# brownvc/matryodshka

Measured on AMD Instinct MI355X. Metric: novel-view frames/sec, 640x320 ODS->32-sphere MSI infer+render, higher is better.
Workload: dtype f32

## Files before the change

### include/msi_hip.h

```cpp
#ifndef MSI_HIP_H
#define MSI_HIP_H

#include <stddef.h>
#include <stdint.h>

#ifdef __cplusplus
extern "C" {
#endif

#define MSI_OK 0
#define MSI_E_BADARG (-1)
#define MSI_E_LAUNCH (-2)
#define MSI_E_UNSUPPORTED (-3)
#define MSI_E_WORKSPACE (-4)
#define MSI_E_RANGE (-5)

typedef void *msi_stream_t;

const char *msi_version(void);
#define MSI_ABI_VERSION 9
int32_t msi_abi_version(void);
const char *msi_last_error_string(void);
uint32_t msi_crc32c_host(const void *data_host, size_t n, uint32_t crc);

int32_t msi_probe_matrix_rate(int32_t changing_operands, int64_t iterations, int32_t num_workgroups, uint64_t *ticks_device, float *sink_device,
                              msi_stream_t stream);

size_t msi_trig_table_floats(int32_t height, int32_t width);
int msi_build_trig_tables_host(int32_t height, int32_t width, float *out_host);

int msi_preprocess_u8_f32(const uint8_t *in, float *out, size_t n, msi_stream_t stream);
int msi_preprocess_f32(const float *in, float *out, size_t n, msi_stream_t stream);
int msi_preprocess_pair_u8_f32(const uint8_t *in0, const uint8_t *in1, float *out0, float *out1, size_t n,
                               msi_stream_t stream);
int msi_deprocess_f32_u8(const float *in, uint8_t *out, size_t n, int32_t is_depth,
                         msi_stream_t stream);
int msi_deprocess_pair_f32_u8(const float *rgb, const float *depth, uint8_t *out_rgb, uint8_t *out_depth, size_t n,
                              msi_stream_t stream);

int msi_compose_poses_f32(const float *lhs, const float *rhs, float *out, int32_t batch,
                          msi_stream_t stream);

int msi_ods_sphere_sweep_f32(const float *image, const float *pose, const float *intrinsics,
                             const float *depths, const float *trig, int32_t batch,
                             int32_t height, int32_t width, int32_t num_depths, int32_t order,
                             float *psv, int32_t psv_channels, int32_t channel_offset,
                             msi_stream_t stream);

int msi_ods_sphere_sweep_bf16(const float *image, const float *pose, const float *intrinsics,
                              const float *depths, const float *trig, int32_t batch,
                              int32_t height, int32_t width, int32_t num_depths, int32_t order,
                              void *psv_bf16, int32_t psv_channels, int32_t channel_offset,
                              msi_stream_t stream);

int msi_ods_sweep_volume(const float *ref_image, const float *src_image, const float *ref_curr_pose,
                         const float *src_curr_pose, const float *intrinsics, const float *depths, const float *trig,
                         int32_t batch, int32_t height, int32_t width, int32_t num_depths, void *psv, int32_t psv_is_bf16,
                         msi_stream_t stream);
int msi_compose_pose_pair_f32(const float *lhs0, const float *lhs1, const float *rhs, float *out0, float *out1,
                              int32_t batch, msi_stream_t stream);

int msi_assemble_rgba_f32(const float *psv, const float *pred, float *rgba_native,
                          float *blend_weights, float *alphas, int32_t batch, int32_t height,
                          int32_t width, int32_t num_planes, msi_stream_t stream);

int msi_assemble_rgba_bf16psv_f32(const void *psv_bf16, const float *pred, float *rgba_native,
                                  float *blend_weights, float *alphas, int32_t batch, int32_t height,
                                  int32_t width, int32_t num_planes, msi_stream_t stream);

#define MSI_COLOR_BLEND_PSV 0
#define MSI_COLOR_BLEND_BG 1
#define MSI_COLOR_BLEND_BG_PSV 2
#define MSI_COLOR_ALPHA_ONLY 3
int msi_assemble_rgba_color_f32(const void *psv, int32_t psv_is_bf16, const float *pred, int32_t which_color_pred,
                                float *rgba_native, float *blend_weights, float *alphas, float *bg_blend_weights,
                                int32_t batch, int32_t height, int32_t width, int32_t num_planes, msi_stream_t stream);

int msi_resize_bilinear_f32(const float *in, float *out, int32_t batch, int32_t in_h, int32_t in_w,
                            int32_t channels, int32_t out_h, int32_t out_w, msi_stream_t stream);
int msi_assemble_rgba_scaled_f32(const float *psv, const float *weights_alphas, float *rgba_native,
                                 int32_t batch, int32_t height, int32_t width, int32_t num_planes,
                                 msi_stream_t stream);
int msi_hres_layers(const float *ref_image, const float *src_image, const float *ref_curr_pose, const float *src_curr_pose,
                    const float *intrinsics, const float *depths, const float *trig, const float *blend_weights,
                    const float *alphas, int32_t batch, int32_t low_height, int32_t low_width, int32_t height, int32_t width,
                    int32_t num_planes, float *rgba_native, void *layers_out, int32_t format, msi_stream_t stream);

#define MSI_RENDER_STATUS_ORIGIN_OUTSIDE 1
int msi_render_equirect_f32(const float *rgba_native, const float *tgt_pose_rt,
                            const float *tgt_pos, const float *depths, const float *trig,
                            int32_t batch, int32_t height, int32_t width, int32_t num_planes,
                            float *out_rgb, float *out_depth, int32_t *status_device, msi_stream_t stream);
#define MSI_CAMERA_EQUIRECT 0
#define MSI_CAMERA_PINHOLE 1
int msi_render_views_f32(const float *rgba_native, const float *tgt_pose_rt, const float *tgt_pos,
                         const float *intrinsics, const float *depths, const float *trig,
                         int32_t batch, int32_t views, int32_t height, int32_t width, int32_t num_planes,
                         int32_t camera, int32_t out_height, int32_t out_width,
                         float *out_rgb, float *out_depth, int32_t *status_device, msi_stream_t stream);

#define MSI_LAYERS_F32 0
#define MSI_LAYERS_RGBA8 1
#define MSI_LAYERS_RGBA16F 2
int msi_pack_layers(const float *rgba_native, int32_t format, void *packed, int64_t texels, msi_stream_t stream);
int msi_unpack_layers(const void *packed, int32_t format, float *rgba_native, int64_t texels, msi_stream_t stream);
int msi_render_views_packed(const void *layers, int32_t format, const float *tgt_pose_rt, const float *tgt_pos,
                            const float *intrinsics, const float *depths, const float *trig,
                            int32_t batch, int32_t views, int32_t height, int32_t width, int32_t num_planes,
                            int32_t camera, int32_t out_height, int32_t out_width,
                            float *out_rgb, float *out_depth, int32_t *status_device, msi_stream_t stream);
int msi_render_ods_views(const void *layers, int32_t format, const float *tgt_pose_rt, const float *tgt_pos,
                         const float *eye_radius, const float *depths, const float *trig,
                         int32_t batch, int32_t views, int32_t height, int32_t width, int32_t num_planes,
                         int32_t out_height, int32_t out_width,
                         float *out_rgb, float *out_depth, int32_t *status_device, msi_stream_t stream);
int msi_sparse_index_tiles(const void *layers, int32_t format, int32_t batch, int32_t num_planes, int32_t height, int32_t width,
                           int32_t *table_out, int32_t *counts_out, msi_stream_t stream);
int msi_sparse_gather_tiles(const void *layers, int32_t format, const int32_t *table, const int64_t *layer_start, int32_t batch,
                            int32_t num_planes, int32_t height, int32_t width, void *pool_out, msi_stream_t stream);
int msi_sparse_expand(const void *pool, const int32_t *table, const int64_t *layer_start, int32_t format, int32_t batch,
                      int32_t num_planes, int32_t height, int32_t width, void *layers_out, msi_stream_t stream);
int msi_render_views_sparse(const void *pool, const int32_t *table, const int64_t *layer_start, int32_t format,
                            const float *tgt_pose_rt, const float *tgt_pos, const float *intrinsics, const float *eye_radius,
                            const float *depths, const float *trig, int32_t batch, int32_t views, int32_t height, int32_t width,
                            int32_t num_planes, int32_t camera, int32_t out_height, int32_t out_width, float *out_rgb,
                            float *out_depth, int32_t *status_device, msi_stream_t stream);
int msi_hres_index_tiles(const float *alphas, int32_t format, int32_t batch, int32_t low_height, int32_t low_width,
                         int32_t height, int32_t width, int32_t num_planes,
                         int32_t *table_out, int32_t *counts_out, msi_stream_t stream);
int msi_hres_layers_sparse(const float *ref_image, const float *src_image, const float *ref_curr_pose, const float *src_curr_pose,
                           const float *intrinsics, const float *depths, const float *trig, const float *blend_weights,
                           const float *alphas, int32_t batch, int32_t low_height, int32_t low_width, int32_t height, int32_t width,
                           int32_t num_planes, const int32_t *table, const int64_t *layer_start, void *pool_out, int32_t format,
                           msi_stream_t stream);
int msi_project_layers_f32(const float *rgba_native, const float *tgt_pose_rt,
                           const float *tgt_pos, const float *depths, const float *trig,
                           int32_t batch, int32_t height, int32_t width, int32_t num_planes,
                           float *out_layers, int32_t *status_device, msi_stream_t stream);

int msi_render_ods_f32(const float *rgba_native, const float *pose, const float *intrinsics,
                       const float *depths, const float *trig, int32_t batch, int32_t height,
                       int32_t width, int32_t num_planes, int32_t order, float *out_rgb,
                       int32_t *status_device, msi_stream_t stream);
int msi_render_perspective_f32(const float *rgba_native, const float *pose, const float *tgt_pos,
                               const float *depths, int32_t batch, int32_t height, int32_t width,
                               int32_t num_planes, int32_t tgt_height, int32_t tgt_width, float *out_rgb,
                               int32_t *status_device, msi_stream_t stream);

int msi_perspective_plane_sweep_f32(const float *image, const float *pose, const float *intrinsics,
                                    const float *depths, int32_t batch, int32_t height, int32_t width,
                                    int32_t num_depths, float *psv, int32_t psv_channels,
                                    int32_t channel_offset, msi_stream_t stream);
int msi_perspective_sweep_volume_bf16(const float *ref_image, const float *src_image, const float *ref_curr_pose,
                                      const float *src_curr_pose, const float *intrinsics, const float *depths,
                                      int32_t batch, int32_t height, int32_t width, int32_t num_depths,
                                      void *psv_bf16, msi_stream_t stream);
int msi_mpi_render_f32(const float *rgba_native, const float *tgt_pose, const float *intrinsics,
                       const float *intrinsics_inv, const float *depths, int32_t batch, int32_t height,
                       int32_t width, int32_t num_planes, float *out_rgb, msi_stream_t stream);
int msi_mpi_render_views(const void *layers, int32_t format, const float *tgt_pose, const float *intrinsics,
                         const float *tgt_intrinsics_inv, const float *depths, int32_t batch, int32_t views, int32_t height,
                         int32_t width, int32_t num_planes, int32_t out_height, int32_t out_width, float *out_rgb,
                         float *out_depth, msi_stream_t stream);

int msi_cube_render_views(const void *layers, int32_t format, const float *tgt_pose_rt, const float *tgt_pos,
                          const float *tgt_intrinsics, const float *stack_intrinsics, const float *depths, const float *trig,
                          int32_t batch, int32_t views, int32_t face_size, int32_t num_planes, int32_t camera,
                          int32_t out_height, int32_t out_width, float *out_rgb, float *out_depth, int32_t *status_device,
                          msi_stream_t stream);
int msi_equirect_to_cube_f32(const float *image, const float *intrinsics, int32_t batch, int32_t height, int32_t width,
                             int32_t channels, int32_t face_size, float *out, msi_stream_t stream);

#define MSI_SCORE_F32 0
#define MSI_SCORE_U8 1
#define MSI_SCORE_RAW 0
#define MSI_SCORE_IMAGE 1
#define MSI_SCORE_DEPTH 2
#define MSI_SCORE_MSE 1u
#define MSI_SCORE_MAE 2u
#define MSI_SCORE_SSIM 4u
size_t msi_score_workspace_bytes(int32_t n_pairs, int32_t height, int32_t width, int32_t channels);
int msi_score_images(const void *pred, const void *target, int32_t dtype, int32_t transform, int32_t quantize, int32_t n_pairs,
                     int32_t group, int32_t height, int32_t width, int32_t channels, const double *row_weights, double max_val,
                     uint32_t metrics, double *out, void *workspace, size_t workspace_bytes, msi_stream_t stream);

typedef struct msi_net_desc {
  int32_t batch, height, width;
  int32_t in_channels;
  int32_t num_outputs;
  int32_t ngf;
  int32_t coord_net;
  int32_t dtype;
} msi_net_desc;

#define MSI_DTYPE_F32 0
#define MSI_DTYPE_BF16 1

#define MSI_NET_NUM_LAYERS 18

typedef struct msi_layer_info {
  char name[16];
  int32_t kind;
  int32_t cin, cout;
  int32_t has_coord;
  int32_t stride, rate;
  int32_t in_h, in_w, out_h, out_w;
  uint64_t param_offset;
  uint64_t param_floats;
  uint64_t raw_offset;
  uint64_t affine_offset;
  uint64_t ln_scale_offset;
} msi_layer_info;

int msi_net_layer_info(const msi_net_desc *desc, int32_t layer, msi_layer_info *out);
size_t msi_net_param_floats(const msi_net_desc *desc);
size_t msi_net_packed_floats(const msi_net_desc *desc);
int msi_net_pack_weights_host(const msi_net_desc *desc, const float *params_host,
                              float *packed_host);
size_t msi_net_workspace_bytes(const msi_net_desc *desc);

typedef struct msi_net_plan msi_net_plan;
#define MSI_NET_OPT_FIXUP_KERNEL 0
#define MSI_NET_OPT_TAILSPLIT 1
#define MSI_NET_OPT_BIGTILE 2
#define MSI_NET_OPT_HEAD_FUSE_LN 3
#define MSI_NET_OPT_NUM_CUS 4
#define MSI_NET_OPT_F32_TILE 5
#define MSI_NET_OPT_F32_TILE_MASK 6
#define MSI_NET_OPT_APPLY_AHEAD 7
#define MSI_NET_OPT_HALO 8
#define MSI_NET_OPT_HALO_SKIP 9
#define MSI_NET_OPT_UNIFORM_SPLIT 10
#define MSI_NET_OPT_BF16_STAGE_RAW 11
#define MSI_NET_OPT_SPLIT_OVERHEAD 12
#define MSI_NET_OPT_BF16_WAVES 13
#define MSI_NET_OPT_F32_SPLIT3 14
#define MSI_NET_OPT_F32_SPLIT_F16 15
#define MSI_NET_OPT_X3_TILE8 16
#define MSI_NET_OPT_X3_ROWPAR 17
#define MSI_NET_OPT_COUNT 18
int msi_net_plan_create(const msi_net_desc *desc, msi_net_plan **out_plan);
void msi_net_plan_destroy(msi_net_plan *plan);
int msi_net_plan_set_option(msi_net_plan *plan, int32_t option, int32_t value);
size_t msi_net_plan_workspace_bytes(const msi_net_plan *plan);
int32_t msi_net_plan_layer_is_normalized(const msi_net_plan *plan, int32_t layer);
int32_t msi_net_plan_layer_kernel(const msi_net_plan *plan, int32_t layer, char *name, size_t name_bytes, int32_t *nblocks,
                                  int32_t *nsplit_tiles);
int32_t msi_net_plan_layer_params(const msi_net_plan *plan, int32_t layer, void *out, size_t bytes, size_t *needed);
#define MSI_NET_STATUS_APPLY_AHEAD_TIMEOUT 1
#define MSI_NET_STATUS_LN_OVERFLOW 2
#define MSI_NET_STATUS_LN_UNDERFLOW 4
#define MSI_NET_STATUS_F16_SPLIT_RANGE 8
int32_t msi_net_plan_status(const msi_net_plan *plan, const void *workspace, msi_stream_t stream, int32_t *status_bits);
int32_t msi_net_plan_calibrate(const msi_net_plan *plan, float *packed, const void *net_input, void *workspace, size_t workspace_bytes,
                               msi_stream_t stream, int32_t *layers_changed);
int msi_net_plan_forward(const msi_net_plan *plan, const float *packed, const void *net_input, float *pred,
                         void *workspace, size_t workspace_bytes, msi_stream_t stream);

int msi_net_plan_forward_rgba(const msi_net_plan *plan, const float *packed, const void *net_input, float *rgba_native,
                              float *blend_weights, float *alphas, float *pred, void *workspace, size_t workspace_bytes,
                              msi_stream_t stream, void *event_after_convs);

int msi_net_plan_forward_layers(const msi_net_plan *plan, const float *packed, const void *net_input, float *rgba_native,
                                void *layers_out, int32_t format, float *blend_weights, float *alphas, float *pred,
                                void *workspace, size_t workspace_bytes, msi_stream_t stream, void *event_after_convs);

int msi_net_forward_f32(const msi_net_desc *desc, const float *packed, const float *net_input,
                        float *pred, void *workspace, size_t workspace_bytes,
                        msi_stream_t stream);
int msi_net_forward_bf16(const msi_net_desc *desc, const float *packed, const void *net_input_bf16,
                         float *pred, void *workspace, size_t workspace_bytes,
                         msi_stream_t stream);

#ifdef __cplusplus
}
#endif
#endif
```

### matryodshka_amd/_native.py

```python
import ctypes
import os
from ctypes import POINTER, Structure, c_char, c_char_p, c_float, c_int32, c_size_t, c_uint64, c_void_p

_HERE = os.path.dirname(os.path.abspath(__file__))
LIB_PATH = os.path.join(_HERE, "libmsi_hip.so")

MSI_OK = 0
MSI_NET_NUM_LAYERS = 18
RENDER_STATUS_ORIGIN_OUTSIDE = 1
MSI_CAMERA_EQUIRECT, MSI_CAMERA_PINHOLE = 0, 1
MSI_LAYERS_F32, MSI_LAYERS_RGBA8, MSI_LAYERS_RGBA16F = 0, 1, 2
MSI_SCORE_F32, MSI_SCORE_U8 = 0, 1
MSI_SCORE_RAW, MSI_SCORE_IMAGE, MSI_SCORE_DEPTH = 0, 1, 2
MSI_SCORE_MSE, MSI_SCORE_MAE, MSI_SCORE_SSIM = 1, 2, 4
MSI_ABI_VERSION = 9


class MsiError(RuntimeError):
    pass


class NetDesc(Structure):
    _fields_ = [("batch", c_int32), ("height", c_int32), ("width", c_int32),
                ("in_channels", c_int32), ("num_outputs", c_int32), ("ngf", c_int32),
                ("coord_net", c_int32), ("dtype", c_int32)]


MSI_DTYPE_F32, MSI_DTYPE_BF16 = 0, 1
NET_OPT_FIXUP_KERNEL, NET_OPT_TAILSPLIT, NET_OPT_BIGTILE, NET_OPT_HEAD_FUSE_LN, NET_OPT_NUM_CUS = 0, 1, 2, 3, 4
NET_OPT_F32_TILE, NET_OPT_F32_TILE_MASK, NET_OPT_APPLY_AHEAD, NET_OPT_HALO, NET_OPT_HALO_SKIP = 5, 6, 7, 8, 9
NET_OPT_UNIFORM_SPLIT, NET_OPT_BF16_STAGE_RAW, NET_OPT_SPLIT_OVERHEAD, NET_OPT_BF16_WAVES, NET_OPT_F32_SPLIT3 = 10, 11, 12, 13, 14
NET_OPT_F32_SPLIT_F16 = 15
NET_OPT_X3_TILE8 = 16
NET_OPT_X3_ROWPAR = 17
NET_STATUS_F16_SPLIT_RANGE = 8


class LayerInfo(Structure):
    _fields_ = [("name", c_char * 16), ("kind", c_int32), ("cin", c_int32), ("cout", c_int32),
                ("has_coord", c_int32), ("stride", c_int32), ("rate", c_int32),
                ("in_h", c_int32), ("in_w", c_int32), ("out_h", c_int32), ("out_w", c_int32),
                ("param_offset", c_uint64), ("param_floats", c_uint64),
                ("raw_offset", c_uint64), ("affine_offset", c_uint64), ("ln_scale_offset", c_uint64)]


_P = c_void_p
_I = c_int32

SIGNATURES = {
    "msi_version": (c_char_p, []),
    "msi_abi_version": (c_int32, []),
    "msi_last_error_string": (c_char_p, []),
    "msi_crc32c_host": (ctypes.c_uint32, [_P, c_size_t, ctypes.c_uint32]),
    "msi_probe_matrix_rate": (_I, [_I, ctypes.c_int64, _I, _P, _P, _P]),
    "msi_trig_table_floats": (c_size_t, [_I, _I]),
    "msi_build_trig_tables_host": (_I, [_I, _I, _P]),
    "msi_preprocess_u8_f32": (_I, [_P, _P, c_size_t, _P]),
    "msi_preprocess_pair_u8_f32": (_I, [_P, _P, _P, _P, c_size_t, _P]),
    "msi_deprocess_pair_f32_u8": (_I, [_P, _P, _P, _P, c_size_t, _P]),
    "msi_preprocess_f32": (_I, [_P, _P, c_size_t, _P]),
    "msi_deprocess_f32_u8": (_I, [_P, _P, c_size_t, _I, _P]),
    "msi_compose_poses_f32": (_I, [_P, _P, _P, _I, _P]),
    "msi_ods_sphere_sweep_f32": (_I, [_P, _P, _P, _P, _P, _I, _I, _I, _I, _I, _P, _I, _I, _P]),
    "msi_ods_sphere_sweep_bf16": (_I, [_P, _P, _P, _P, _P, _I, _I, _I, _I, _I, _P, _I, _I, _P]),
    "msi_ods_sweep_volume": (_I, [_P, _P, _P, _P, _P, _P, _P, _I, _I, _I, _I, _P, _I, _P]),
    "msi_compose_pose_pair_f32": (_I, [_P, _P, _P, _P, _P, _I, _P]),
    "msi_assemble_rgba_f32": (_I, [_P, _P, _P, _P, _P, _I, _I, _I, _I, _P]),
    "msi_assemble_rgba_bf16psv_f32": (_I, [_P, _P, _P, _P, _P, _I, _I, _I, _I, _P]),
    "msi_assemble_rgba_color_f32": (_I, [_P, _I, _P, _I, _P, _P, _P, _P, _I, _I, _I, _I, _P]),
    "msi_resize_bilinear_f32": (_I, [_P, _P, _I, _I, _I, _I, _I, _I, _P]),
    "msi_assemble_rgba_scaled_f32": (_I, [_P, _P, _P, _I, _I, _I, _I, _P]),
    "msi_hres_layers": (_I, [_P, _P, _P, _P, _P, _P, _P, _P, _P, _I, _I, _I, _I, _I, _I, _P, _P, _I, _P]),
    "msi_render_equirect_f32": (_I, [_P, _P, _P, _P, _P, _I, _I, _I, _I, _P, _P, _P, _P]),
    "msi_render_views_f32": (_I, [_P, _P, _P, _P, _P, _P, _I, _I, _I, _I, _I, _I, _I, _I, _P, _P, _P, _P]),
    "msi_pack_layers": (_I, [_P, _I, _P, ctypes.c_int64, _P]),
    "msi_unpack_layers": (_I, [_P, _I, _P, ctypes.c_int64, _P]),
    "msi_render_views_packed": (_I, [_P, _I, _P, _P, _P, _P, _P, _I, _I, _I, _I, _I, _I, _I, _I, _P, _P, _P, _P]),
    "msi_render_ods_views": (_I, [_P, _I, _P, _P, _P, _P, _P, _I, _I, _I, _I, _I, _I, _I, _P, _P, _P, _P]),
    "msi_sparse_index_tiles": (_I, [_P, _I, _I, _I, _I, _I, _P, _P, _P]),
    "msi_sparse_gather_tiles": (_I, [_P, _I, _P, _P, _I, _I, _I, _I, _P, _P]),
    "msi_sparse_expand": (_I, [_P, _P, _P, _I, _I, _I, _I, _I, _P, _P]),
    "msi_render_views_sparse": (_I, [_P, _P, _P, _I, _P, _P, _P, _P, _P, _P, _I, _I, _I, _I, _I, _I, _I, _I, _P, _P, _P, _P]),
    "msi_hres_index_tiles": (_I, [_P, _I, _I, _I, _I, _I, _I, _I, _P, _P, _P]),
    "msi_hres_layers_sparse": (_I, [_P, _P, _P, _P, _P, _P, _P, _P, _P, _I, _I, _I, _I, _I, _I, _P, _P, _P, _I, _P]),
    "msi_project_layers_f32": (_I, [_P, _P, _P, _P, _P, _I, _I, _I, _I, _P, _P, _P]),
    "msi_render_ods_f32": (_I, [_P, _P, _P, _P, _P, _I, _I, _I, _I, _I, _P, _P, _P]),
    "msi_render_perspective_f32": (_I, [_P, _P, _P, _P, _I, _I, _I, _I, _I, _I, _P, _P, _P]),
    "msi_perspective_plane_sweep_f32": (_I, [_P, _P, _P, _P, _I, _I, _I, _I, _P, _I, _I, _P]),
    "msi_perspective_sweep_volume_bf16": (_I, [_P, _P, _P, _P, _P, _P, _I, _I, _I, _I, _P, _P]),
    "msi_mpi_render_f32": (_I, [_P, _P, _P, _P, _P, _I, _I, _I, _I, _P, _P]),
    "msi_mpi_render_views": (_I, [_P, _I, _P, _P, _P, _P, _I, _I, _I, _I, _I, _I, _I, _P, _P, _P]),
    "msi_cube_render_views": (_I, [_P, _I, _P, _P, _P, _P, _P, _P, _I, _I, _I, _I, _I, _I, _I, _P, _P, _P, _P]),
    "msi_equirect_to_cube_f32": (_I, [_P, _P, _I, _I, _I, _I, _I, _P, _P]),
    "msi_score_workspace_bytes": (c_size_t, [_I, _I, _I, _I]),
    "msi_score_images": (_I, [_P, _P, _I, _I, _I, _I, _I, _I, _I, _I, _P, ctypes.c_double, ctypes.c_uint32, _P, _P, c_size_t, _P]),
    "msi_net_layer_info": (_I, [POINTER(NetDesc), _I, POINTER(LayerInfo)]),
    "msi_net_param_floats": (c_size_t, [POINTER(NetDesc)]),
    "msi_net_packed_floats": (c_size_t, [POINTER(NetDesc)]),
    "msi_net_pack_weights_host": (_I, [POINTER(NetDesc), _P, _P]),
    "msi_net_workspace_bytes": (c_size_t, [POINTER(NetDesc)]),
    "msi_net_plan_create": (_I, [POINTER(NetDesc), POINTER(c_void_p)]),
    "msi_net_plan_destroy": (None, [_P]),
    "msi_net_plan_set_option": (_I, [_P, _I, _I]),
    "msi_net_plan_workspace_bytes": (c_size_t, [_P]),
    "msi_net_plan_layer_is_normalized": (_I, [_P, _I]),
    "msi_net_plan_layer_kernel": (_I, [_P, _I, _P, c_size_t, POINTER(c_int32), POINTER(c_int32)]),
    "msi_net_plan_layer_params": (_I, [_P, _I, _P, c_size_t, POINTER(c_size_t)]),
    "msi_net_plan_status": (_I, [_P, _P, _P, POINTER(c_int32)]),
    "msi_net_plan_calibrate": (_I, [_P, _P, _P, _P, c_size_t, _P, POINTER(c_int32)]),
    "msi_net_plan_forward": (_I, [_P, _P, _P, _P, _P, c_size_t, _P]),
    "msi_net_plan_forward_rgba": (_I, [_P, _P, _P, _P, _P, _P, _P, _P, c_size_t, _P, _P]),
    "msi_net_plan_forward_layers": (_I, [_P, _P, _P, _P, _P, _I, _P, _P, _P, _P, c_size_t, _P, _P]),
    "msi_net_forward_f32": (_I, [POINTER(NetDesc), _P, _P, _P, _P, c_size_t, _P]),
    "msi_net_forward_bf16": (_I, [POINTER(NetDesc), _P, _P, _P, _P, c_size_t, _P]),
}


def _load():
    import torch
    if not os.path.exists(LIB_PATH):
        raise ImportError(
            "matryodshka_amd: %s is missing -- build it with `python -m matryodshka_amd.build` "
            "(or __graft_entry__.build()).  There is no CPU fallback." % LIB_PATH)
    lib = ctypes.CDLL(LIB_PATH)
    for name, (res, args) in SIGNATURES.items():
        try:
            fn = getattr(lib, name)
        except AttributeError:
            raise ImportError("matryodshka_amd: %s does not export %s" % (LIB_PATH, name))
        fn.restype = res
        fn.argtypes = args
    if lib.msi_abi_version() != MSI_ABI_VERSION:
        raise ImportError("matryodshka_amd: %s has ABI version %d, this binding is written for %d -- rebuild it "
                          "(python -m matryodshka_amd.build --force)" % (LIB_PATH, lib.msi_abi_version(), MSI_ABI_VERSION))
    return lib


lib = _load()


def last_error():
    return lib.msi_last_error_string().decode("utf-8", "replace")


class NetPlan(object):

    def __init__(self, desc, options=None):
        h = c_void_p()
        check(lib.msi_net_plan_create(desc, ctypes.byref(h)), "msi_net_plan_create")
        self.handle = h
        self._destroy = lib.msi_net_plan_destroy
        for key, value in (options or {}).items():
            self.set_option(key, value)

    def set_option(self, key, value):
        check(lib.msi_net_plan_set_option(self.handle, int(key), int(value)), "msi_net_plan_set_option")

    def workspace_bytes(self):
        return lib.msi_net_plan_workspace_bytes(self.handle)

    def layer_kernel(self, layer):
        buf = ctypes.create_string_buffer(96)
        nb, ns = c_int32(0), c_int32(0)
        check(lib.msi_net_plan_layer_kernel(self.handle, int(layer), ctypes.cast(buf, c_void_p), 96, ctypes.byref(nb), ctypes.byref(ns)),
              "msi_net_plan_layer_kernel")
        return buf.value.decode(), int(nb.value), int(ns.value)

    def layer_params(self, layer):
        n = c_size_t(0)
        check(lib.msi_net_plan_layer_params(self.handle, int(layer), None, 0, ctypes.byref(n)), "msi_net_plan_layer_params")
        buf = ctypes.create_string_buffer(n.value)
        check(lib.msi_net_plan_layer_params(self.handle, int(layer), ctypes.cast(buf, c_void_p), n.value, None), "msi_net_plan_layer_params")
        return buf.raw

    def kernels(self):
        return [self.layer_kernel(i) for i in range(18)]

    def __del__(self):
        h, self.handle = getattr(self, "handle", None), None
        if h:
            self._destroy(h)


def check(rc, what):
    if rc != MSI_OK:
        raise MsiError("%s failed (code %d): %s" % (what, rc, last_error()))
```

### matryodshka_amd/csrc/cnn.hip

```cpp
#include "cnn_plan.h"

namespace msi_cnn {

int device_cu_count() {
  int dev = 0;
  hipDeviceProp_t prop;
  if (hipGetDevice(&dev) != hipSuccess || hipGetDeviceProperties(&prop, dev) != hipSuccess || prop.multiProcessorCount <= 0) {
    (void)hipGetLastError();
    return DEFAULT_CUS;
  }
  return prop.multiProcessorCount;
}

int launch_conv(const LayerLaunch &Q, const ConvParams &p, hipStream_t stream) {
  const ConvVariant &V = Q.variant;
  int rc;
  switch (V.family) {
    case CONV_IGEMM: rc = launch_igemm(Q, p, stream); break;
    case CONV_HALO: case CONV_HALO_S2: case CONVT_HALO: rc = launch_halo_f32(Q, p, stream); break;
    case CONV_HALO_X3: case CONV_HALO8_X3: case CONV_HALO_S2_X3: case CONV_HALO8_S2_X3: case CONVT_HALO_X3: case CONVT_HALO8_X3: rc = launch_x3(Q, p, stream); break;
    case CONV_HALO_BF16: case CONV_HALO_BF16_S2: case CONVT_HALO_BF16: rc = launch_bf16_halo(Q, p, stream); break;
    default: return msi::fail(MSI_E_UNSUPPORTED, "conv: unknown kernel family %d", V.family);
  }
  if (rc || Q.nfix == 0 || p.tile_cnt != nullptr) return rc;
  const int mode = V.family == CONV_IGEMM ? V.mode : (V.is_convt() ? MODE_CONVT : MODE_CONV);
  return launch_fixup(V.bm, V.bn, mode, V.family == CONV_IGEMM && V.bf16 && mode != MODE_HEAD, Q.nfix, V.is_convt() ? 2 : 1, p, stream);
}

}

#if defined(MSI_CONV_TIMING) || defined(MSI_DEBUG_STATS)
static unsigned long long *g_timing_buf = nullptr;
static int g_timing_layer = -1;
extern "C" int msi_debug_conv_occupancy(int lds_bytes) {
  return msi_cnn::debug_conv_occupancy(lds_bytes);
}
extern "C" void msi_debug_conv_timing(void *device_buffer, int layer) {
  g_timing_buf = static_cast<unsigned long long *>(device_buffer);
  g_timing_layer = layer;
}
#endif

extern "C" {

#ifdef MSI_DEBUG_SUMS
extern "C" long long msi_debug_sums_offset(const msi_net_plan *plan, int layer) { return (long long)plan->net.layers[layer].sums_off; }
extern "C" long long msi_debug_partial_offset(const msi_net_plan *plan) { return (long long)plan->net.partial_off; }
#endif
static int run_layers(const msi_net_plan *plan, const float *packed, const void *net_input, float *pred,
                      void *workspace, size_t workspace_bytes, msi_stream_t stream_, int nlayers) {
  MSI_REQUIRE(plan, "net_forward: null plan");
  const msi_net_desc *desc = &plan->desc;
  const Net &net = plan->net;
  const int bf16 = desc->dtype == MSI_DTYPE_BF16;
  MSI_REQUIRE(packed && net_input && workspace, "net_forward: null pointer");
  if (workspace_bytes < net.ws_bytes)
    return msi::fail(MSI_E_WORKSPACE, "net_forward: workspace %zu B < required %zu B", workspace_bytes,
                     net.ws_bytes);
  if (desc->batch == 0) return MSI_OK;
  hipStream_t stream = msi::as_stream(stream_);
  char *ws = static_cast<char *>(workspace);
  {
    const size_t n16 = net.zero_bytes / 16;
    int rc0 = launch_zero(ws + net.zero_off, n16, stream);
    if (rc0) return rc0;
  }
  int *cnt = reinterpret_cast<int *>(ws + net.cnt_off);
  for (int li = 0; li < nlayers; ++li) {
    const Layer &L = net.layers[li];
    const LayerLaunch &Q = plan->launch[li];
    ConvParams p = Q.p;
    auto src_ptr = [&](int s) -> const char * {
      if (s < 0) return static_cast<const char *>(net_input);
      return ws + (bf16 ? net.layers[s].act_off : net.layers[s].raw_off);
    };
    p.x0 = src_ptr(L.src0);
    p.x1 = L.src1 >= 0 ? src_ptr(L.src1) : p.x0;
    p.wpk = reinterpret_cast<const char *>(packed + L.packed_off);
    p.coord_bias = L.has_coord ? packed + L.coord_off : nullptr;
    p.bias = L.kind == MODE_HEAD ? packed + L.gamma_off : nullptr;
    if (Q.fuse_ln) {
      const Layer &S = net.layers[L.src0];
      p.ln_sums = reinterpret_cast<const long long *>(ws + S.sums_off);
      p.ln_gamma = packed + S.gamma_off;
      p.ln_beta = packed + S.beta_off;
    }
    p.y = L.kind == MODE_HEAD ? pred : reinterpret_cast<float *>(ws + L.raw_off);
    p.sums = L.kind == MODE_HEAD ? nullptr : reinterpret_cast<long long *>(ws + L.sums_off);
    auto scl_of = [&](int li2) { return reinterpret_cast<const double *>(packed + net.layers[li2].lnscl_off); };
    p.ln_scl = L.kind == MODE_HEAD ? nullptr : scl_of(li);
    p.ln_scl_src = L.src0 >= 0 ? scl_of(L.src0) : nullptr;
    p.ln_scl_src1 = L.src1 >= 0 ? scl_of(L.src1) : nullptr;
    p.status = reinterpret_cast<int *>(ws + net.err_off);
    p.partial = reinterpret_cast<float *>(ws + net.partial_off);
    p.tile_cnt = Q.inlaunch ? cnt + (size_t)li * CONV_SLOTS_PER_CU * plan->num_cus : nullptr;
#if defined(MSI_CONV_TIMING) || defined(MSI_DEBUG_STATS)
    p.dbg = (li == g_timing_layer) ? g_timing_buf : nullptr;
#endif
    auto raw_source = [&](int s, bool second) {
      const Layer &S = net.layers[s];
      if (!second) {
        if (bf16) p.x0 = ws + S.raw_off;
        p.ln_sums = reinterpret_cast<const long long *>(ws + S.sums_off); p.ln_gamma = packed + S.gamma_off; p.ln_beta = packed + S.beta_off;
      } else {
        if (bf16) p.x1 = ws + S.raw_off;
        p.ln_sums1 = reinterpret_cast<const long long *>(ws + S.sums_off); p.ln_gamma1 = packed + S.gamma_off; p.ln_beta1 = packed + S.beta_off;
      }
    };
    const ConvVariant &V = Q.variant;
    if (V.is_convt()) {
      if (p.halo_apply & 1) raw_source(L.src0, false);
      if (p.halo_apply & 2) raw_source(L.src1, true);
    } else if (V.apply) {
      raw_source(L.src0, false);
    }
    if (V.six_product()) p.wpk_x3 = reinterpret_cast<const char *>(packed + (V.planes == 2 ? L.x2_off : L.x3_off));
    int rc = launch_conv(Q, p, stream);
    if (rc) return rc;
    const bool tail_src = bf16 && nlayers == MSI_NET_NUM_LAYERS - 1 && li == net.layers[MSI_NET_NUM_LAYERS - 1].src0;
    if (L.kind != MODE_HEAD && !Q.skip_apply && !tail_src) {
      const size_t per_sample = (size_t)L.out_h * L.out_w * L.cout;
      float *raw = reinterpret_cast<float *>(ws + L.raw_off), *aff = reinterpret_cast<float *>(ws + L.aff_off);
      const size_t lds = (size_t)2 * L.cout * sizeof(float);
      const long long *sums = reinterpret_cast<const long long *>(ws + L.sums_off);
      rc = launch_ln_apply(bf16, Q.ln_blocks, desc->batch, lds, stream, raw, sums, 1.0 / L.ln_count, scl_of(li), p.status, packed + L.gamma_off, packed + L.beta_off,
                           per_sample, L.cout, aff, bf16 ? reinterpret_cast<unsigned short *>(ws + L.act_off) : static_cast<unsigned short *>(nullptr));
      if (rc) return rc;
    }
  }
  return MSI_OK;
}

int32_t msi_net_plan_status(const msi_net_plan *plan, const void *workspace, msi_stream_t stream_, int32_t *status_bits) {
  MSI_REQUIRE(plan && workspace, "net_plan_status: null pointer");
  hipStream_t stream = msi::as_stream(stream_);
  int word = 0;
  hipError_t e = hipMemcpyAsync(&word, static_cast<const char *>(workspace) + plan->net.err_off, sizeof(int), hipMemcpyDeviceToHost, stream);
  if (e == hipSuccess) e = hipStreamSynchronize(stream);
  if (e != hipSuccess) return msi::fail(MSI_E_LAUNCH, "net_plan_status: %s", hipGetErrorString(e));
  if (status_bits) *status_bits = word;
  if (word == 0) return MSI_OK;
  return msi::fail(MSI_E_RANGE, "net_plan_status: 0x%x:%s%s%s", word,
                   (word & STATUS_F16_SPLIT_RANGE) ? " an operand of a layer on the fp16 split exceeded the fp16 range (|x| > 65504): set MSI_NET_OPT_F32_SPLIT_F16 = 0" : "",
                   (word & STATUS_LN_OVERFLOW) ? " a LayerNorm sum left its fixed-point window (raw convolution output far above the scale the weights predict: non-finite or mis-scaled input?)" : "",
                   (word & STATUS_LN_UNDERFLOW) ? " a LayerNorm variance is below the resolution of its fixed-point window (raw convolution output far below the scale the weights predict, or constant)" : "");
}

int32_t msi_net_plan_calibrate(const msi_net_plan *plan, float *packed, const void *net_input, void *workspace, size_t workspace_bytes,
                               msi_stream_t stream_, int32_t *layers_changed) {
  MSI_REQUIRE(plan && packed && net_input && workspace, "net_plan_calibrate: null pointer");
  const Net &net = plan->net;
  const msi_net_desc *desc = &plan->desc;
  hipStream_t stream = msi::as_stream(stream_);
  if (layers_changed) *layers_changed = 0;
  if (desc->batch == 0) return MSI_OK;
  const size_t nwords = (size_t)desc->batch * LN_SHARDS * LN_WORDS;
  std::vector<long long> sums(nwords);
  char *ws = static_cast<char *>(workspace);
  constexpr int NL = MSI_NET_NUM_LAYERS - 1;
  double orig[NL][LN_SCL_DOUBLES];
  hipError_t he = hipSuccess;
  for (int li = 0; li < NL && he == hipSuccess; ++li)
    he = hipMemcpyAsync(orig[li], packed + net.layers[li].lnscl_off, sizeof(orig[li]), hipMemcpyDeviceToHost, stream);
  if (he == hipSuccess) he = hipStreamSynchronize(stream);
  if (he != hipSuccess) return msi::fail(MSI_E_LAUNCH, "net_plan_calibrate: %s", hipGetErrorString(he));
  int touched = 0;
  auto restore = [&]() {
    for (int l = 0; l < touched; ++l)
      (void)hipMemcpyAsync(packed + net.layers[l].lnscl_off, orig[l], sizeof(orig[l]), hipMemcpyHostToDevice, stream);
    (void)hipStreamSynchronize(stream);
  };
  for (int li = 0; li < NL; ++li) {
    const Layer &L = net.layers[li];
    const double *scl = orig[li];
    int e0 = LN_S1_BITS - (int)lrint(log2(scl[0])), e = e0;
    bool settled = false;
    touched = li + 1;
    for (int it = 0; it < 24 && !settled; ++it) {
      const double ns[LN_SCL_DOUBLES] = {ldexp(1.0, LN_S1_BITS - e), ldexp(1.0, LN_S2_BITS - 2 * e), ldexp(1.0, -(LN_S1_BITS - e)), ldexp(1.0, -(LN_S2_BITS - 2 * e))};
      he = hipMemcpyAsync(packed + L.lnscl_off, ns, sizeof(ns), hipMemcpyHostToDevice, stream);
      if (he == hipSuccess) he = hipStreamSynchronize(stream);
      if (he != hipSuccess) { restore(); return msi::fail(MSI_E_LAUNCH, "net_plan_calibrate: %s", hipGetErrorString(he)); }
      int rc = run_layers(plan, packed, net_input, nullptr, workspace, workspace_bytes, stream_, li + 1);
      if (rc) { restore(); return rc; }
      int word = 0;
      he = hipMemcpyAsync(sums.data(), ws + L.sums_off, nwords * sizeof(long long), hipMemcpyDeviceToHost, stream);
      if (he == hipSuccess) he = hipMemcpyAsync(&word, ws + net.err_off, sizeof(int), hipMemcpyDeviceToHost, stream);
      if (he == hipSuccess) he = hipStreamSynchronize(stream);
      if (he != hipSuccess) { restore(); return msi::fail(MSI_E_LAUNCH, "net_plan_calibrate: %s", hipGetErrorString(he)); }
      if (word & STATUS_LN_OVERFLOW) { e += 12; if (e > 120) break; continue; }
      double rmin = 1e300, rmax = 0.0, amin = 1e300, amax = 0.0;
      for (int b = 0; b < desc->batch; ++b) {
        double h2 = 0.0;
        for (int sh = 0; sh < LN_SHARDS; ++sh)
          h2 += (double)sums[((size_t)b * LN_SHARDS + sh) * LN_WORDS + 1];
        const bool under = h2 * h2 < LN_UNDERFLOW_UNITS_SQ * (L.ln_count / 1024.0 + 1.0);
        const double ms = h2 * ns[3] / L.ln_count;
        const double r = sqrt(ms > 0.0 ? ms : 0.0);
        if (r > 0.0) { amin = r < amin ? r : amin; amax = r > amax ? r : amax; }
        if (r > 0.0 && !under) { rmin = r < rmin ? r : rmin; rmax = r > rmax ? r : rmax; }
      }
      if (rmax > 0.0) {
        const int ec = (int)lrint(0.5 * (log2(rmax) + log2(rmin)));
        if (ec > e + 1 || ec < e - 1) { e = ec; continue; }
        settled = true;
      } else if (amax > 0.0) {
        const int ec = (int)lrint(0.5 * (log2(amax) + log2(amin)));
        if (ec > e + 1 || ec < e - 1) e = ec; else e -= 12;
        if (e < -120) break;
      } else { e -= 12; if (e < -120) break; }
    }
    if (!settled) {
      restore();
      if (layers_changed) *layers_changed = 0;
      return msi::fail(MSI_E_RANGE, "net_plan_calibrate: layer %s has no finite, non-constant raw output to centre a LayerNorm window on (non-finite input or weights, "
                       "or a constant frame?); the windows are unchanged", L.name);
    }
    if (e != e0 && layers_changed) ++*layers_changed;
  }
  return MSI_OK;
}

int msi_net_plan_forward(const msi_net_plan *plan, const float *packed, const void *net_input, float *pred,
                         void *workspace, size_t workspace_bytes, msi_stream_t stream_) {
  MSI_REQUIRE(pred, "net_forward: null pointer");
  return run_layers(plan, packed, net_input, pred, workspace, workspace_bytes, stream_, MSI_NET_NUM_LAYERS);
}

static int forward_fused_tail(const char *who, const msi_net_plan *plan, const float *packed, const void *net_input, float *rgba_native,
                              void *layers_out, int32_t format, float *blend_weights, float *alphas, float *pred, void *workspace,
                              size_t workspace_bytes, msi_stream_t stream_, void *event_after_convs) {
  MSI_REQUIRE(plan, "%s: null plan", who);
  const msi_net_desc *desc = &plan->desc;
  const Net &net = plan->net;
  const Layer &H = net.layers[MSI_NET_NUM_LAYERS - 1];
  const int nd = desc->num_outputs / 2;
  const int bf16 = desc->dtype == MSI_DTYPE_BF16;
  if ((!bf16 && !plan->launch[MSI_NET_NUM_LAYERS - 1].fuse_ln) || (bf16 && !plan->opt[MSI_NET_OPT_HEAD_FUSE_LN]) ||
      H.c0 > 64 || H.c0 % 4 != 0 || desc->num_outputs != 2 * nd || nd % 4 != 0 || nd > 64 || desc->in_channels != 6 * nd ||
      ((long)desc->height * desc->width) % HA_TP != 0)
    return msi::fail(MSI_E_UNSUPPORTED, "%s: fused tail needs a blend_psv network (in = 6 D, out = 2 D, "
                     "D %% 4 == 0, D <= 64, ngf <= 64, HEAD_FUSE_LN on)", who);
  MSI_REQUIRE(rgba_native || layers_out, "%s: null pointer", who);
  MSI_REQUIRE(!layers_out || (reinterpret_cast<uintptr_t>(layers_out) & 15) == 0, "%s: layers_out is not 16-byte aligned", who);
  const int ng = (nd + HA_LG - 1) / HA_LG;
  if (nd % ng != 0 || (nd / ng) % 4 != 0 || (ng > 1 && bf16 && (nd / ng) % 8 != 0))
    return msi::fail(MSI_E_UNSUPPORTED, "%s: D = %d does not split into layer groups of a multiple of %d", who, nd, bf16 ? 8 : 4);
  int rc = run_layers(plan, packed, net_input, nullptr, workspace, workspace_bytes, stream_, MSI_NET_NUM_LAYERS - 1);
  if (rc || desc->batch == 0) return rc;
  hipStream_t stream = msi::as_stream(stream_);
  if (event_after_convs) {
    hipError_t e = hipEventRecord(static_cast<hipEvent_t>(event_after_convs), stream);
    if (e != hipSuccess) return msi::fail(MSI_E_LAUNCH, "%s: %s", who, hipGetErrorString(e));
  }
  char *ws = static_cast<char *>(workspace);
  const Layer &S = net.layers[H.src0];
  HeadAsmParams q;
  q.x = reinterpret_cast<const float *>(ws + S.raw_off);
  q.wpk = packed + H.packed_off;
  q.bias = packed + H.gamma_off;
  float *aff = reinterpret_cast<float *>(ws + S.aff_off);
  rc = launch_ln_finish(desc->batch, stream, reinterpret_cast<const long long *>(ws + S.sums_off), 1.0 / S.ln_count,
                        reinterpret_cast<const double *>(packed + S.lnscl_off), reinterpret_cast<int *>(ws + net.err_off),
                        packed + S.gamma_off, packed + S.beta_off, S.cout, aff, bf16);
  if (rc) return rc;
  q.aff = aff;
  q.psv = net_input;
  q.rgba = reinterpret_cast<float4 *>(rgba_native);
  q.layers = layers_out;
  q.bw_out = blend_weights;
  q.al_out = alphas;
  q.pred_out = pred;
  q.C0 = H.c0; q.ksteps = H.ksteps; q.npad = H.npad;
  q.nd = nd; q.hw = desc->height * desc->width;
  q.npix_total = (long)desc->batch * q.hw;
  q.lg = nd / ng;
  q.ng = ng;
  {
    auto magic = [](unsigned d) { return d == 1 ? 0xffffffffu : (unsigned)((1ull << 32) / d); };
    const int vec = bf16 ? 8 : 4;
    const unsigned vpp = (unsigned)((ng == 1 ? 6 * nd : 2 * 3 * q.lg) / vec);
    q.mg_vpp = magic(vpp);
    q.mg_nchunk = magic((unsigned)(q.ksteps * 8));
    q.mg_hw = magic((unsigned)q.hw);
    if (q.npix_total >= (1L << 32)) return msi::fail(MSI_E_UNSUPPORTED, "%s: more than 2^32 pixels per batch", who);
  }
  constexpr int BN = 64;
  size_t r_bytes = (size_t)q.ksteps * (HA_TP + BN) * ROW_BYTES;
  if (r_bytes < (size_t)HA_TP * (6 * q.lg + 1) * sizeof(float)) r_bytes = (size_t)HA_TP * (6 * q.lg + 1) * sizeof(float);
  if (bf16) {
    r_bytes = (size_t)q.ksteps * HA_TP * ROW_BYTES;
    if (r_bytes < (size_t)HA_TP * (3 * q.lg + 1) * sizeof(unsigned)) r_bytes = (size_t)HA_TP * (3 * q.lg + 1) * sizeof(unsigned);
  }
  const size_t lds = 2 * 64 * 4 + 64 + ((r_bytes + 15) & ~(size_t)15) + (size_t)HA_TP * (2 * q.lg + 1) * sizeof(float);
  const long ntile = q.npix_total / HA_TP;
  if (((ntile + 7) / 8) * 8 * ng >= (1L << 31)) return msi::fail(MSI_E_UNSUPPORTED, "%s: too many pixel tiles for one launch", who);
  return launch_head_assemble(bf16, layers_out ? format : MSI_LAYERS_F32, (unsigned)(((ntile + 7) / 8) * 8 * ng), lds, stream, q);
}

int msi_net_plan_forward_rgba(const msi_net_plan *plan, const float *packed, const void *net_input, float *rgba_native,
                              float *blend_weights, float *alphas, float *pred, void *workspace, size_t workspace_bytes,
                              msi_stream_t stream_, void *event_after_convs) {
  return forward_fused_tail("net_forward_rgba", plan, packed, net_input, rgba_native, nullptr, MSI_LAYERS_F32, blend_weights, alphas, pred,
                            workspace, workspace_bytes, stream_, event_after_convs);
}

int msi_net_plan_forward_layers(const msi_net_plan *plan, const float *packed, const void *net_input, float *rgba_native,
                                void *layers_out, int32_t format, float *blend_weights, float *alphas, float *pred, void *workspace,
                                size_t workspace_bytes, msi_stream_t stream_, void *event_after_convs) {
  MSI_REQUIRE(!layers_out || format == MSI_LAYERS_RGBA8 || format == MSI_LAYERS_RGBA16F,
              "net_forward_layers: unknown format %d (layers_out is MSI_LAYERS_RGBA8 or MSI_LAYERS_RGBA16F)", format);
  MSI_REQUIRE(rgba_native || layers_out, "net_forward_layers: null pointer");
  return forward_fused_tail("net_forward_layers", plan, packed, net_input, rgba_native, layers_out, format, blend_weights, alphas, pred,
                            workspace, workspace_bytes, stream_, event_after_convs);
}

size_t msi_net_workspace_bytes(const msi_net_desc *desc) {
  msi_net_plan *pl = nullptr;
  if (msi_net_plan_create(desc, &pl)) return 0;
  const size_t n = pl->net.ws_bytes;
  msi_net_plan_destroy(pl);
  return n;
}

static int forward_once(const msi_net_desc *desc, const float *packed, const void *net_input, float *pred,
                        void *workspace, size_t workspace_bytes, msi_stream_t stream) {
  msi_net_plan *pl = nullptr;
  int rc = msi_net_plan_create(desc, &pl);
  if (rc) return rc;
  rc = msi_net_plan_forward(pl, packed, net_input, pred, workspace, workspace_bytes, stream);
  msi_net_plan_destroy(pl);
  return rc;
}

int msi_net_forward_f32(const msi_net_desc *desc, const float *packed, const float *net_input,
                        float *pred, void *workspace, size_t workspace_bytes, msi_stream_t stream) {
  MSI_REQUIRE(desc && desc->dtype == MSI_DTYPE_F32, "net_forward_f32: desc->dtype must be MSI_DTYPE_F32");
  return forward_once(desc, packed, net_input, pred, workspace, workspace_bytes, stream);
}

int msi_net_forward_bf16(const msi_net_desc *desc, const float *packed, const void *net_input_bf16,
                         float *pred, void *workspace, size_t workspace_bytes, msi_stream_t stream) {
  MSI_REQUIRE(desc && desc->dtype == MSI_DTYPE_BF16, "net_forward_bf16: desc->dtype must be MSI_DTYPE_BF16");
  return forward_once(desc, packed, net_input_bf16, pred, workspace, workspace_bytes, stream);
}

}
```

### matryodshka_amd/csrc/cnn_device.h

```cpp
#pragma once
#include <cmath>
#include <cstdint>
#include <cstdio>
#include <cstdlib>
#include <cstring>
#include <new>
#include <type_traits>
#include <vector>

#include "msi_common.h"

namespace msi_cnn {


typedef float f32x16 __attribute__((ext_vector_type(16)));
typedef float v4f __attribute__((ext_vector_type(4)));
typedef __attribute__((address_space(3))) void lds_void;

constexpr int BK = 32;
constexpr int ROW_BYTES = BK * 4;
#ifndef MSI_NSTAGE
#define MSI_NSTAGE 2
#endif
constexpr int NSTAGE = MSI_NSTAGE;
constexpr int NPAD_ALIGN = 128;
constexpr int COORD_CLASSES = 5;
[[maybe_unused]] constexpr unsigned OOB = 0x80000000u;
constexpr int DEFAULT_CUS = 256;
constexpr int MAX_SPLIT = 8;
constexpr int CONV_SLOTS_PER_CU = 5;
constexpr double LN_EPS = 1e-12;
constexpr int LN_SHARDS = 64, LN_WORDS = 2;
constexpr int LN_S1_BITS = 24, LN_S2_BITS = 16;
constexpr int LN_SCL_DOUBLES = 4;
constexpr double LN_UNDERFLOW_UNITS_SQ = 1e12;
enum { STATUS_APPLY_AHEAD_TIMEOUT = 1 , STATUS_LN_OVERFLOW = 2, STATUS_LN_UNDERFLOW = 4, STATUS_F16_SPLIT_RANGE = 8 };
constexpr int HEAD_MAX_C = 256;

enum { MODE_CONV = 0, MODE_CONVT = 1, MODE_HEAD = 2 };

struct ConvParams {
  const char *x0, *x1;
  const char *wpk;
  const char *wpk_x3;
  const float *coord_bias;
  int cb_stride;
  const double *ln_scl;
  const double *ln_scl_src, *ln_scl_src1;
  int *status;
  const long long *ln_sums;
  const float *ln_gamma, *ln_beta;
  double ln_inv_n;
  const long long *ln_sums1;
  const float *ln_gamma1, *ln_beta1;
  double ln_inv_n1;
  int halo_apply;
  const float *bias;
  float *y;
  long long *sums;
  float *partial;
  int *tile_cnt;
  int tiles_m, tiles_n, ntiles;
  int n_main, split0, split;
  int nb_main;
  int C0, C1;
  int Hin, Win, Hout, Wout, Cout, npad;
  int Mh, Mw;
  unsigned mg_mw, mg_tm, mg_tn, mg_nc, mg_sp0, mg_sp;
  int ntaps, cpt0, cpt1, ksteps;
  int stride, rate, pad_t, pad_l;
  int mode, wrap, nclass;
  int halo_tx;
  unsigned mg_htx;
  int halo_xor;
  int row_par;
#if defined(MSI_CONV_TIMING) || defined(MSI_DEBUG_STATS)
  unsigned long long *dbg;
#endif
};

enum ConvFamily {
  CONV_IGEMM = 0,
  CONV_HALO, CONV_HALO_S2, CONVT_HALO,
  CONV_HALO_X3, CONV_HALO8_X3, CONV_HALO_S2_X3, CONV_HALO8_S2_X3, CONVT_HALO_X3, CONVT_HALO8_X3,
  CONV_HALO_BF16, CONV_HALO_BF16_S2, CONVT_HALO_BF16,
};
struct ConvVariant {
  int family;
  int bm, bn;
  int mode, bf16;
  int rate;
  int apply;
  int planes;
  int waves;
  bool is_halo() const { return family != CONV_IGEMM; }
  bool is_convt_f32() const { return family == CONVT_HALO || family == CONVT_HALO_X3 || family == CONVT_HALO8_X3; }
  bool is_convt() const { return is_convt_f32() || family == CONVT_HALO_BF16; }
  bool six_product() const { return family >= CONV_HALO_X3 && family <= CONVT_HALO8_X3; }
  bool tile8() const { return family == CONV_HALO8_X3 || family == CONV_HALO8_S2_X3 || family == CONVT_HALO8_X3; }
};

struct LayerLaunch {
  ConvParams p;
  ConvVariant variant;
  int nblocks, nfix;
  int inlaunch;
  int fuse_ln;
  int skip_apply;
  unsigned ln_blocks;
};

constexpr int HA_TP = 32;
#ifndef MSI_HA_LG
#define MSI_HA_LG 32
#endif
constexpr int HA_LG = MSI_HA_LG;

struct HeadAsmParams {
  const float *x;
  const float *wpk;
  const float *bias;
  const float *aff;
  const void *psv;
  float4 *rgba;
  float *bw_out, *al_out;
  float *pred_out;
  int C0, ksteps, npad, nd, hw;
  int lg, ng;
  unsigned mg_vpp, mg_nchunk, mg_hw;
  long npix_total;
  void *layers;
};

int launch_conv(const LayerLaunch &Q, const ConvParams &p, hipStream_t stream);
int launch_igemm(const LayerLaunch &Q, const ConvParams &p, hipStream_t stream);
int launch_fixup(int bm, int bn, int mode, int raw16, unsigned grid_x, unsigned grid_y, const ConvParams &p, hipStream_t stream);
int launch_halo_f32(const LayerLaunch &Q, const ConvParams &p, hipStream_t stream);
int launch_x3(const LayerLaunch &Q, const ConvParams &p, hipStream_t stream);
int launch_bf16_halo(const LayerLaunch &Q, const ConvParams &p, hipStream_t stream);
int launch_zero(void *p, size_t n16, hipStream_t stream);
int launch_ln_finish(int batch, hipStream_t stream, const long long *sums, double inv_n, const double *scl, int *status, const float *gamma, const float *beta, int C,
                     float *aff, int raw16);
int launch_ln_apply(int bf16out, unsigned blocks, int batch, size_t lds, hipStream_t stream, float *x, const long long *sums, double inv_n, const double *scl, int *status,
                    const float *gamma, const float *beta, size_t per_sample, int C, float *aff, unsigned short *yb);
int launch_head_assemble(int bf16in, int format, unsigned grid_x, size_t lds, hipStream_t stream, const HeadAsmParams &q);
int debug_conv_occupancy(int lds_bytes);

constexpr int vkey(int family, int a = 0, int b = 0, int c = 0, int d = 0, int e = 0) { return ((((family * 16 + a) * 16 + b) * 16 + c) * 16 + d) * 16 + e; }

inline int set_max_lds(const void *fn, int lds, unsigned long long &done, const char *what) {
  int dev = 0;
  if (hipGetDevice(&dev) != hipSuccess) dev = 0;
  const bool tracked = dev >= 0 && dev < 64;
  if (tracked && ((done >> dev) & 1ull)) return MSI_OK;
  hipError_t e = hipFuncSetAttribute(fn, hipFuncAttributeMaxDynamicSharedMemorySize, lds);
  if (e != hipSuccess) return msi::fail(MSI_E_LAUNCH, "%s: %s", what, hipGetErrorString(e));
  if (tracked) done |= 1ull << dev;
  return MSI_OK;
}

template <auto KERNEL, int LDS, int THREADS = 256>
int launch_kernel(unsigned nblocks, const ConvParams &p, hipStream_t stream, const char *what) {
  if constexpr (LDS > 65536) {
    static thread_local unsigned long long done = 0;
    int rc0 = set_max_lds(reinterpret_cast<const void *>(KERNEL), LDS, done, what);
    if (rc0) return rc0;
  }
  hipLaunchKernelGGL(KERNEL, dim3(nblocks), dim3(THREADS), LDS, stream, p);
  return msi::check_launch(what);
}

template <int N> using IC = std::integral_constant<int, N>;
}
using namespace msi_cnn;

namespace {

template <int MODE>
__device__ __forceinline__ int tap_delta(int v, int parity, int rate, bool wrapt) {
  if (MODE == MODE_CONV) return v * rate;
  if (MODE == MODE_CONVT) return wrapt ? -v : (v == 0 ? 0 : (parity ? 1 : -1));
  return 0;
}

__device__ __forceinline__ unsigned udiv_magic(unsigned x, unsigned d, unsigned mg) {
  unsigned q = __umulhi(x, mg);
  if (x - q * d >= d) ++q;
  return q;
}

__device__ __forceinline__ int halo_row(const ConvParams &p, int tyi, int r, int rows_per_tile) {
  return p.row_par ? (tyi >> 1) * (2 * rows_per_tile) + (tyi & 1) + 2 * r : tyi * rows_per_tile + r;
}

__device__ __forceinline__ int xcd_contiguous(int bid, int n) {
  const int q = n >> 3, r = n & 7, xcd = bid & 7, local = bid >> 3;
  return (xcd < r ? xcd * (q + 1) : r * (q + 1) + (xcd - r) * q) + local;
}
struct TileWork { int t, k0, ks, slot, k1; bool full; };
__device__ __forceinline__ TileWork tile_work(const ConvParams &p, int n) {
  TileWork w = {0, 0, 0, 0, n, true};
  const int bid = (int)blockIdx.x;
  if (bid < p.nb_main && p.split0 == 1) {
    w.t = xcd_contiguous(bid, p.n_main);
  } else {
    unsigned mg;
    int tbase, r, sp;
    if (bid < p.nb_main) { sp = p.split0; mg = p.mg_sp0; r = bid; tbase = 0; }
    else { sp = p.split; mg = p.mg_sp; r = bid - p.nb_main; tbase = p.n_main; }
    const int tl = (int)udiv_magic((unsigned)r, (unsigned)sp, mg);
    w.ks = r - tl * sp;
    w.t = tbase + tl;
    w.k0 = (int)udiv_magic((unsigned)(w.ks * n), (unsigned)sp, mg);
    w.k1 = (int)udiv_magic((unsigned)((w.ks + 1) * n), (unsigned)sp, mg);
    w.slot = bid - (p.split0 == 1 ? p.nb_main : 0);
  }
  w.full = (w.k0 == 0) & (w.k1 == n);
  return w;
}

enum { TILE_NO_CLASS = 0,
       TILE_CLASSES = 1,
       TILE_ROW_PARITY = 2 };
struct TileIndex { int tile_m, tile_n, cls, b; };
template <int CLASS_MODE = TILE_NO_CLASS>
__device__ __forceinline__ TileIndex tile_index(const ConvParams &p, int t) {
  int tile_m, tile_n, cls = 0, b;
  int r = t;
  if (CLASS_MODE == TILE_CLASSES) {
    const int q0 = (int)udiv_magic((unsigned)r, (unsigned)p.nclass, p.mg_nc);
    cls = r - q0 * p.nclass; r = q0;
  } else if (CLASS_MODE == TILE_ROW_PARITY) {
    cls = r & 1; r >>= 1;
  }
  const int q1 = (int)udiv_magic((unsigned)r, (unsigned)p.tiles_m, p.mg_tm);
  tile_m = r - q1 * p.tiles_m; r = q1;
  const int q2 = (int)udiv_magic((unsigned)r, (unsigned)p.tiles_n, p.mg_tn);
  tile_n = r - q2 * p.tiles_n;
  b = q2;
  return TileIndex{tile_m, tile_n, cls, b};
}

__device__ __forceinline__ float msi_tanh(float x) {
  const float xa = fminf(fabsf(x), 15.0f);
  const float t = __builtin_amdgcn_exp2f(xa * 2.8853900817779268f);
  const float r = (t - 1.0f) * __builtin_amdgcn_rcpf(t + 1.0f);
  return x != x ? x : __builtin_copysignf(r, x);
}

__device__ __forceinline__ int coord_class(int mw, int Mw) {
  return mw < 2 ? mw : (mw >= Mw - 2 ? 3 + (mw - (Mw - 2)) : 2);
}

template <int N>
__device__ __forceinline__ void wait_vmcnt() {
  asm volatile("s_waitcnt vmcnt(%0)" ::"n"(N) : "memory");
}

template <int OFF>
__device__ __forceinline__ v4f lds_read128(unsigned addr) {
  v4f v;
  if constexpr (OFF < 65536) {
    asm volatile("ds_read_b128 %0, %1 offset:%2" : "=v"(v) : "v"(addr), "n"(OFF) : "memory");
  } else {
    asm volatile("ds_read_b128 %0, %1 offset:%2" : "=v"(v) : "v"(addr + (OFF & ~0xffff)), "n"(OFF & 0xffff) : "memory");
  }
  return v;
}
template <int N>
__device__ __forceinline__ void wait_lgkm(v4f &x, v4f &y) {
  asm volatile("s_waitcnt lgkmcnt(%2)" : "+v"(x), "+v"(y) : "n"(N) : "memory");
}
template <int N, int MT, int NT>
__device__ __forceinline__ void wait_lgkm_frag(v4f (&a)[MT], v4f (&b)[NT]) {
  static_assert((MT == 1 || MT == 2 || MT == 4) && (NT == 1 || NT == 2), "fragment shapes of the conv kernels");
  if constexpr (MT == 1 && NT == 1) asm volatile("s_waitcnt lgkmcnt(%2)" : "+v"(a[0]), "+v"(b[0]) : "n"(N) : "memory");
  else if constexpr (MT == 2 && NT == 1) asm volatile("s_waitcnt lgkmcnt(%3)" : "+v"(a[0]), "+v"(a[1]), "+v"(b[0]) : "n"(N) : "memory");
  else if constexpr (MT == 1 && NT == 2) asm volatile("s_waitcnt lgkmcnt(%3)" : "+v"(a[0]), "+v"(b[0]), "+v"(b[1]) : "n"(N) : "memory");
  else if constexpr (MT == 2 && NT == 2) asm volatile("s_waitcnt lgkmcnt(%4)" : "+v"(a[0]), "+v"(a[1]), "+v"(b[0]), "+v"(b[1]) : "n"(N) : "memory");
  else if constexpr (MT == 4 && NT == 1) asm volatile("s_waitcnt lgkmcnt(%5)" : "+v"(a[0]), "+v"(a[1]), "+v"(a[2]), "+v"(a[3]), "+v"(b[0]) : "n"(N) : "memory");
  else asm volatile("s_waitcnt lgkmcnt(%6)" : "+v"(a[0]), "+v"(a[1]), "+v"(a[2]), "+v"(a[3]), "+v"(b[0]), "+v"(b[1]) : "n"(N) : "memory");
}

__device__ __forceinline__ float wave_sum(float x) {
#define MSI_DPP_ADD(CTRL, ROWMASK)                                                                                     \
  x += __builtin_bit_cast(float, __builtin_amdgcn_update_dpp(0, __builtin_bit_cast(int, x), CTRL, ROWMASK, 0xf, true))
  MSI_DPP_ADD(0xB1, 0xf);
  MSI_DPP_ADD(0x4E, 0xf);
  MSI_DPP_ADD(0x141, 0xf);
  MSI_DPP_ADD(0x140, 0xf);
  MSI_DPP_ADD(0x142, 0xa);
  MSI_DPP_ADD(0x143, 0xc);
#undef MSI_DPP_ADD
  return __builtin_bit_cast(float, __builtin_amdgcn_readlane(__builtin_bit_cast(int, x), 63));
}

__device__ __forceinline__ double wave_sum_f64(double x) {
#define MSI_DPP_ADD64(CTRL, ROWMASK)                                                                                   \
  {                                                                                                                    \
    const long long b_ = __builtin_bit_cast(long long, x);                                                             \
    const int lo_ = __builtin_amdgcn_update_dpp(0, (int)b_, CTRL, ROWMASK, 0xf, true);                                 \
    const int hi_ = __builtin_amdgcn_update_dpp(0, (int)(b_ >> 32), CTRL, ROWMASK, 0xf, true);                         \
    x += __builtin_bit_cast(double, ((long long)hi_ << 32) | (unsigned)lo_);                                           \
  }
  MSI_DPP_ADD64(0xB1, 0xf) MSI_DPP_ADD64(0x4E, 0xf) MSI_DPP_ADD64(0x141, 0xf) MSI_DPP_ADD64(0x140, 0xf)
  MSI_DPP_ADD64(0x142, 0xa) MSI_DPP_ADD64(0x143, 0xc)
#undef MSI_DPP_ADD64
  const long long b = __builtin_bit_cast(long long, x);
  const int lo = __builtin_amdgcn_readlane((int)b, 63), hi = __builtin_amdgcn_readlane((int)(b >> 32), 63);
  return __builtin_bit_cast(double, ((long long)hi << 32) | (unsigned)lo);
}

__device__ __forceinline__ void ln_atomic_add(long long *dst, double x_scaled, int *status) {
  const double MAGIC = 6755399441055744.0;
  if (!(fabs(x_scaled) < 2251799813685248.0 )) {
    if (status) __hip_atomic_fetch_or(status, STATUS_LN_OVERFLOW, __ATOMIC_RELAXED, __HIP_MEMORY_SCOPE_AGENT);
    return;
  }
  const double t = x_scaled + MAGIC;
  const long long v = __builtin_bit_cast(long long, t) - __builtin_bit_cast(long long, MAGIC);
  __hip_atomic_fetch_add(dst, v, __ATOMIC_RELAXED, __HIP_MEMORY_SCOPE_AGENT);
}

struct LnShard { long long w0, w1; };
__device__ __forceinline__ LnShard ln_shard_load(const long long *sums, int tid) {
  LnShard r = {0, 0};
  if (tid < 64) {
    const long long *s = sums + (size_t)tid * LN_WORDS;
    r.w0 = s[0]; r.w1 = s[1];
  }
  return r;
}
template <bool PRE>
__device__ __forceinline__ void ln_mean_inv_impl(const long long *sums, LnShard pre, double inv_n, const double *scl, int *status, double *s_stat, int tid) {
  static_assert(LN_SHARDS == 64, "one shard per lane of wave 0");
  const double inv_s1 = scl[2], inv_s2 = scl[3];
  if (tid < 64) {
    long long w0 = pre.w0, w1 = pre.w1;
    if constexpr (!PRE) {
      const long long *s = sums + (size_t)tid * LN_WORDS;
      w0 = s[0]; w1 = s[1];
    }
    const double h1 = wave_sum_f64((double)w0), h2 = wave_sum_f64((double)w1);
    if (tid == 0) {
      const double S1 = h1 * inv_s1, S2 = h2 * inv_s2;
      if (status && h2 * h2 < LN_UNDERFLOW_UNITS_SQ * (1.0 / (inv_n * 1024.0) + 1.0))
        __hip_atomic_fetch_or(status, STATUS_LN_UNDERFLOW, __ATOMIC_RELAXED, __HIP_MEMORY_SCOPE_AGENT);
      const double mu = S1 * inv_n;
      double var = S2 * inv_n - mu * mu;
      var = var > 0.0 ? var : 0.0;
      const double x = var + LN_EPS, hx = 0.5 * x;
      double r = __builtin_amdgcn_rsq(x);
      r = r * (1.5 - hx * r * r);
      r = r * (1.5 - hx * r * r);
      s_stat[0] = mu;
      s_stat[1] = r;
    }
  }
  __syncthreads();
}
__device__ __forceinline__ void ln_mean_inv(const long long *sums, double inv_n, const double *scl, int *status, double *s_stat, int tid) {
  ln_mean_inv_impl<false>(sums, LnShard{0, 0}, inv_n, scl, status, s_stat, tid);
}
__device__ __forceinline__ void ln_mean_inv_pre(LnShard pre, double inv_n, const double *scl, int *status, double *s_stat, int tid) {
  ln_mean_inv_impl<true>(nullptr, pre, inv_n, scl, status, s_stat, tid);
}
struct LnAffine { float inv, mu_hi, mu_lo; };
__device__ __forceinline__ LnAffine ln_affine_read(const double *s_stat) {
  const double mu = s_stat[0];
  LnAffine a;
  a.inv = (float)s_stat[1];
  a.mu_hi = (float)mu;
  a.mu_lo = (float)(mu - (double)a.mu_hi);
  __syncthreads();
  return a;
}
__device__ __forceinline__ void ln_scale_shift(const LnAffine &a, const v4f &g4, const v4f &be4, v4f &s4, v4f &t4) {
  s4 = a.inv * g4;
  const v4f nh = {-a.mu_hi, -a.mu_hi, -a.mu_hi, -a.mu_hi}, nl = {-a.mu_lo, -a.mu_lo, -a.mu_lo, -a.mu_lo};
  t4 = __builtin_elementwise_fma(nl, s4, __builtin_elementwise_fma(nh, s4, be4));
}

typedef unsigned u32x4_t __attribute__((ext_vector_type(4)));

#ifndef MSI_HANDOFF_FENCE
#define MSI_HANDOFF_FENCE 0
#endif
#ifndef MSI_HANDOFF_AUX
#define MSI_HANDOFF_AUX 16
#endif
__device__ __forceinline__ void handoff_release() {
  if (MSI_HANDOFF_FENCE & 1) __builtin_amdgcn_fence(__ATOMIC_RELEASE, "agent");
}
__device__ __forceinline__ void handoff_acquire() {
  if (MSI_HANDOFF_FENCE & 2) __builtin_amdgcn_fence(__ATOMIC_ACQUIRE, "agent");
}

template <int MT, int NT, int AUX>
__device__ __forceinline__ void dump_acc(const f32x16 (&acc)[MT][NT], __amdgpu_buffer_rsrc_t rsrc, int tid) {
#pragma unroll
  for (int i = 0; i < MT; ++i)
#pragma unroll
    for (int j = 0; j < NT; ++j)
#pragma unroll
      for (int g = 0; g < 4; ++g) {
        const v4f v = {acc[i][j][4 * g], acc[i][j][4 * g + 1], acc[i][j][4 * g + 2], acc[i][j][4 * g + 3]};
        __builtin_amdgcn_raw_buffer_store_b128(__builtin_bit_cast(u32x4_t, v), rsrc,
                                               (unsigned)((((i * NT + j) * 4 + g) * 256 + tid) * 16), 0, AUX);
      }
}

template <int MT, int NT, int AUX>
__device__ __forceinline__ void sum_slabs(f32x16 (&acc)[MT][NT], __amdgpu_buffer_rsrc_t rsrc, int nsp, int slab_bytes, int tid) {
  for (int s = 0; s < nsp; ++s) {
    v4f t[MT][NT][4];
#pragma unroll
    for (int i = 0; i < MT; ++i)
#pragma unroll
      for (int j = 0; j < NT; ++j)
#pragma unroll
        for (int g = 0; g < 4; ++g)
          t[i][j][g] = __builtin_bit_cast(v4f, (u32x4_t)__builtin_amdgcn_raw_buffer_load_b128(
              rsrc, (unsigned)((((i * NT + j) * 4 + g) * 256 + tid) * 16), s * slab_bytes, AUX));
#pragma unroll
    for (int i = 0; i < MT; ++i)
#pragma unroll
      for (int j = 0; j < NT; ++j)
#pragma unroll
        for (int g = 0; g < 4; ++g) {
          if (s == 0) {
            acc[i][j][4 * g] = t[i][j][g].x; acc[i][j][4 * g + 1] = t[i][j][g].y;
            acc[i][j][4 * g + 2] = t[i][j][g].z; acc[i][j][4 * g + 3] = t[i][j][g].w;
          } else {
            acc[i][j][4 * g] += t[i][j][g].x; acc[i][j][4 * g + 1] += t[i][j][g].y;
            acc[i][j][4 * g + 2] += t[i][j][g].z; acc[i][j][4 * g + 3] += t[i][j][g].w;
          }
        }
  }
}

struct ConvStamps {
#ifdef MSI_CONV_TIMING
  unsigned long long ts0, ts0r, ts1, ts2;
  __device__ __forceinline__ void begin() { ts0 = __builtin_amdgcn_s_memtime(); ts0r = __builtin_amdgcn_s_memrealtime(); }
  __device__ __forceinline__ void loop() { ts1 = __builtin_amdgcn_s_memtime(); }
  __device__ __forceinline__ void tail() { ts2 = __builtin_amdgcn_s_memtime(); }
  __device__ __forceinline__ void write(const ConvParams &p, int tid) const {
    if (p.dbg && tid == 0) {
      unsigned long long *o = p.dbg + (size_t)blockIdx.x * 24;
      o[0] = ts0; o[1] = ts1; o[2] = ts2; o[3] = __builtin_amdgcn_s_memtime(); o[22] = ts0r; o[23] = __builtin_amdgcn_s_memrealtime();
      o[4] = __builtin_amdgcn_s_getreg(4 | (31 << 11));
      o[5] = __builtin_amdgcn_s_getreg(20 | (31 << 11));
    }
  }
#else
  __device__ __forceinline__ void begin() {}
  __device__ __forceinline__ void loop() {}
  __device__ __forceinline__ void tail() {}
  __device__ __forceinline__ void write(const ConvParams &, int) const {}
#endif
};

template <int MT, int NT>
__device__ __forceinline__ bool splitk_arrive(const ConvParams &p, const f32x16 (&acc)[MT][NT], const TileWork &w, char *smem, int tid) {
  constexpr int TILE = MT * NT * 16 * 256, SLAB = TILE * 4;
  const __amdgpu_buffer_rsrc_t rsrc_p = __builtin_amdgcn_make_buffer_rsrc((void *)(p.partial + (size_t)w.slot * TILE), 0, SLAB, 0x00020000);
  if (p.tile_cnt == nullptr) {
    dump_acc<MT, NT, 0>(acc, rsrc_p, tid);
    return false;
  }
  dump_acc<MT, NT, MSI_HANDOFF_AUX>(acc, rsrc_p, tid);
  const int nsp = w.t < p.n_main ? p.split0 : p.split;
  asm volatile("s_waitcnt vmcnt(0)" ::: "memory");
  handoff_release();
  __syncthreads();
  int *s_old = reinterpret_cast<int *>(smem);
  if (tid == 0)
    *s_old = __hip_atomic_fetch_add(p.tile_cnt + (w.t - (p.split0 == 1 ? p.n_main : 0)), 1, __ATOMIC_RELAXED, __HIP_MEMORY_SCOPE_AGENT);
  __syncthreads();
  return *s_old == nsp - 1;
}
template <int MT, int NT>
__device__ __forceinline__ void splitk_sum(const ConvParams &p, f32x16 (&acc)[MT][NT], const TileWork &w, int tid) {
  constexpr int TILE = MT * NT * 16 * 256, SLAB = TILE * 4;
  const int nsp = w.t < p.n_main ? p.split0 : p.split;
  handoff_acquire();
  const __amdgpu_buffer_rsrc_t rsrc_t = __builtin_amdgcn_make_buffer_rsrc((void *)(p.partial + (size_t)(w.slot - w.ks) * TILE), 0, nsp * SLAB, 0x00020000);
  sum_slabs<MT, NT, MSI_HANDOFF_AUX>(acc, rsrc_t, nsp, SLAB, tid);
  __syncthreads();
}

constexpr int EPI_STAGE_BYTES = 48 * 1024;
#ifndef MSI_EPI_NT
#define MSI_EPI_NT 0
#endif
#ifdef MSI_CONV_TIMING
#define MSI_STAMP(k) { if (p.dbg && tid == 0) p.dbg[(size_t)blockIdx.x * 24 + (k)] = __builtin_amdgcn_s_memtime(); }
#else
#define MSI_STAMP(k)
#endif
template <int BM, int BN, int MODE, int RAW16, bool CB, bool STAGED, int WR>
__device__ __forceinline__ void emit_whole_tile(const ConvParams &p, f32x16 (&acc)[BM / (32 * WR)][BN / 64], int tile_m, int tile_n, int cls,
                                                int b, int tid, const v4f (&cb_pre)[4], bool use_pre, float pivot, float raw_mul,
                                                double scl_s1, double scl_s2, char *stage) {
  constexpr int MT = BM / (32 * WR), NT = BN / 64, NG = NT * 4, YSZ = RAW16 ? 2 : 4;
  constexpr int ROWB = NT * 32 * YSZ, PITCH = ROWB + 16, NP = ROWB / 16, PPI = 64 / NP, NRD = 32 / PPI;
  constexpr bool FITS = 2 * WR * MT * 32 * PITCH <= EPI_STAGE_BYTES;
  typedef float v2f __attribute__((ext_vector_type(2)));
  typedef _Float16 h2_t __attribute__((ext_vector_type(2)));
  typedef unsigned u2_t __attribute__((ext_vector_type(2)));
  const int lane = tid & 63, wave = tid >> 6, wm = wave >> 1, wn = wave & 1, half = lane >> 5;
  const int ph = cls >> 1, pw = cls & 1;
  const int mtot = p.Mh * p.Mw;
  const bool want_stats = p.sums != nullptr;
  const float pv_s = pivot * raw_mul;
  const v2f rm = {raw_mul, raw_mul}, pv = {pv_s, pv_s};
  const int nbw = tile_n * BN + wn * (NT * 32), nb0 = nbw + 4 * half;
  const size_t sample_bytes = (size_t)(MODE == MODE_CONVT ? p.Hout * p.Wout : mtot) * p.Cout * YSZ;
  constexpr bool staged = STAGED;
  static_assert(!STAGED || FITS, "staging strips");
  const int tyi = p.halo_tx ? (int)udiv_magic((unsigned)tile_m, (unsigned)p.halo_tx, p.mg_htx) : 0;
  const int txi = tile_m - tyi * p.halo_tx;
  MSI_STAMP(16)
  char *yp[MT];
  const float *cbp[MT];
#pragma unroll
  for (int i = 0; i < MT; ++i) {
    yp[i] = nullptr; cbp[i] = nullptr;
    if (CB || !staged) {
      int m = tile_m * BM + wm * (MT * 32) + i * 32 + (lane & 31);
      if (p.halo_tx) {
        const int local = wm * (MT * 32) + i * 32 + (lane & 31);
        m = halo_row(p, tyi, local >> 4, BM / 16) * p.Mw + txi * 16 + ((local & 15) ^ (((local >> 4) & 1) * p.halo_xor));
      }
      int mh = 0, mw = 0;
      if (MODE == MODE_CONVT || CB) {
        mh = (int)udiv_magic((unsigned)m, (unsigned)p.Mw, p.mg_mw);
        mw = m - mh * p.Mw;
      }
      const size_t opix = MODE == MODE_CONVT ? ((size_t)b * p.Hout + (2 * mh + ph)) * p.Wout + (2 * mw + pw) : (size_t)b * mtot + m;
      yp[i] = reinterpret_cast<char *>(p.y) + (opix * p.Cout + nb0) * YSZ;
      if (CB) cbp[i] = p.coord_bias + (size_t)(mh * COORD_CLASSES + coord_class(mw, p.Mw)) * p.cb_stride + nb0;
    }
  }
  char *wst = stage + wave * (MT * 32 * PITCH);
  const int slot = p.halo_tx ? ((lane & 16) | ((lane & 15) ^ (((lane >> 4) & 1) * p.halo_xor))) : (lane & 31);
  char *wp = wst + slot * PITCH + half * (4 * YSZ);
  v2f s1v[4] = {}, s2v[4] = {};
#pragma unroll
  for (int i = 0; i < MT; ++i) {
    v2f ya[NG], yc[NG];
#pragma unroll
    for (int q = 0; q < NG; ++q) {
      ya[q] = v2f{acc[i][q >> 2][4 * (q & 3)], acc[i][q >> 2][4 * (q & 3) + 1]};
      yc[q] = v2f{acc[i][q >> 2][4 * (q & 3) + 2], acc[i][q >> 2][4 * (q & 3) + 3]};
    }
    if (CB) {
      v4f cb[NG];
#pragma unroll
      for (int q = 0; q < NG; ++q)
        cb[q] = (MT == 1 && NT == 1 && use_pre) ? cb_pre[q & 3] : *reinterpret_cast<const v4f *>(cbp[i] + (q >> 2) * 32 + 8 * (q & 3));
#pragma unroll
      for (int q = 0; q < NG; ++q) { ya[q] += v2f{cb[q].x, cb[q].y}; yc[q] += v2f{cb[q].z, cb[q].w}; }
    }
    if (RAW16) {
#pragma unroll
      for (int q = 0; q < NG; ++q) { ya[q] *= rm; yc[q] *= rm; }
    }
    u2_t hw[NG];
    if (RAW16) {
#pragma unroll
      for (int q = 0; q < NG; ++q) {
        const h2_t lo = {(_Float16)ya[q].x, (_Float16)ya[q].y}, hi = {(_Float16)yc[q].x, (_Float16)yc[q].y};
        hw[q] = u2_t{__builtin_bit_cast(unsigned, lo), __builtin_bit_cast(unsigned, hi)};
      }
    }
#pragma unroll
    for (int q = 0; q < NG; ++q) {
      char *dst = staged ? wp + i * (32 * PITCH) : yp[i];
      if (RAW16) *reinterpret_cast<u2_t *>(dst + ((q >> 2) * 32 + 8 * (q & 3)) * 2) = hw[q];
      else *reinterpret_cast<v4f *>(dst + ((q >> 2) * 32 + 8 * (q & 3)) * 4) = v4f{ya[q].x, ya[q].y, yc[q].x, yc[q].y};
    }
    if (want_stats) {
#pragma unroll
      for (int q = 0; q < NG; ++q) { ya[q] -= pv; yc[q] -= pv; }
#pragma unroll
      for (int q = 0; q < NG; ++q) { s1v[q & 3] += ya[q]; s1v[q & 3] += yc[q]; }
#pragma unroll
      for (int q = 0; q < NG; ++q) {
        s2v[q & 3] = __builtin_elementwise_fma(ya[q], ya[q], s2v[q & 3]);
        s2v[q & 3] = __builtin_elementwise_fma(yc[q], yc[q], s2v[q & 3]);
      }
    }
  }
  MSI_STAMP(21)
  const v2f t1 = (s1v[0] + s1v[1]) + (s1v[2] + s1v[3]), t2 = (s2v[0] + s2v[1]) + (s2v[2] + s2v[3]);
  float s1 = t1.x + t1.y, s2 = t2.x + t2.y;
  if (staged) {
    const char *rp = wst + (lane / NP) * PITCH + (lane % NP) * 16;
    v4f pc[MT][NRD];
#pragma unroll
    for (int i = 0; i < MT; ++i)
#pragma unroll
      for (int k = 0; k < NRD; ++k) pc[i][k] = *reinterpret_cast<const v4f *>(rp + (i * 32 + k * PPI) * PITCH);
    const __amdgpu_buffer_rsrc_t rsrc_y = __builtin_amdgcn_make_buffer_rsrc(reinterpret_cast<char *>(p.y) + (size_t)b * sample_bytes, 0, (int)(unsigned)sample_bytes, 0x00020000);
    const int rowb = p.Cout * YSZ;
    int pix0, rowstep, colstep;
    if (p.halo_tx) {
      const int r0 = halo_row(p, tyi, wm * (MT * 2), BM / 16), c0 = txi * 16 + lane / NP;
      if (MODE == MODE_CONVT) { pix0 = (2 * r0 + ph) * p.Wout + 2 * c0 + pw; rowstep = 2 * p.Wout; colstep = 2; }
      else { pix0 = r0 * p.Mw + c0; rowstep = p.row_par ? 2 * p.Mw : p.Mw; colstep = 1; }
    } else {
      pix0 = tile_m * BM + wm * (MT * 32) + lane / NP; rowstep = 16; colstep = 1;
    }
    const unsigned v0 = (unsigned)pix0 * (unsigned)rowb + (unsigned)(nbw * YSZ + (lane % NP) * 16);
#pragma unroll
    for (int i = 0; i < MT; ++i)
#pragma unroll
      for (int k = 0; k < NRD; ++k) {
        const int ro = 2 * i + ((k * PPI) >> 4), co = (k * PPI) & 15;
        __builtin_amdgcn_raw_buffer_store_b128(__builtin_bit_cast(u32x4_t, pc[i][k]), rsrc_y, v0 + (unsigned)((ro * rowstep + co * colstep) * rowb), 0, MSI_EPI_NT ? 2 : 0);
      }
  }
  MSI_STAMP(17)
  if (want_stats) {
    s1 = wave_sum(s1); s2 = wave_sum(s2);
    MSI_STAMP(18)
    if (lane == 0) {
      const double P = (double)pv_s, n = (double)(MT * NT * 16 * 64), a = (double)s1;
      const double u1 = RAW16 ? 16777216.0 : scl_s1, u2 = RAW16 ? 65536.0 : scl_s2;
      if (RAW16 && !(s2 <= 1.0727e9f)) __hip_atomic_fetch_or(p.status, STATUS_LN_OVERFLOW, __ATOMIC_RELAXED, __HIP_MEMORY_SCOPE_AGENT);
      long long *dst = p.sums + ((size_t)b * LN_SHARDS + ((blockIdx.x * 4 + wave) & (LN_SHARDS - 1))) * LN_WORDS;
      ln_atomic_add(dst, (n * P + a) * u1, p.status);
      ln_atomic_add(dst + 1, ((double)s2 + 2.0 * P * a + n * P * P) * u2, p.status);
    }
    MSI_STAMP(19)
  }
}

template <int BM, int BN, int MODE, bool INTERIOR, int RAW16, int WR>
__device__ __forceinline__ void emit_tile_impl(const ConvParams &p, f32x16 (&acc)[BM / (32 * WR)][BN / 64], int tile_m,
                                               int tile_n, int cls, int b, int tid, const v4f (&cb_pre)[4], bool use_pre, char *stage,
                                               float raw_mul_pre) {
  constexpr int MT = BM / (32 * WR), NT = BN / 64;
  const int lane = tid & 63, wave = tid >> 6, wm = wave >> 1, wn = wave & 1, half = lane >> 5;
  const int ph = cls >> 1, pw = cls & 1;
  const int mtot = p.Mh * p.Mw;
  const bool wrapt = MODE == MODE_CONVT && p.wrap != 0;
  const bool vec_ok = (p.Cout & 3) == 0;
  const bool has_cb = MODE == MODE_CONV && p.coord_bias != nullptr;
  const bool want_stats = MODE != MODE_HEAD && p.sums != nullptr;
  const float pivot = __builtin_bit_cast(float, __builtin_amdgcn_readfirstlane(__builtin_bit_cast(int, acc[0][0][0])));
  double scl_s1 = 0.0, scl_s2 = 0.0;
  const bool have_pre = INTERIOR && RAW16 && MODE != MODE_HEAD && raw_mul_pre > 0.f;
  if ((want_stats || RAW16) && !have_pre) { scl_s1 = p.ln_scl[0]; scl_s2 = p.ln_scl[1]; }
  const float raw_mul = have_pre ? raw_mul_pre : RAW16 ? (float)(scl_s1 * (1.0 / 16777216.0)) : 1.f;
  constexpr int YSZ = RAW16 ? 2 : 4;
  float s1 = 0.f, s2 = 0.f, cnt = 0.f;
  if constexpr (INTERIOR && MODE != MODE_HEAD) {
    constexpr bool FITS = 2 * WR * MT * 32 * (NT * 32 * (RAW16 ? 2 : 4) + 16) <= EPI_STAGE_BYTES;
    const size_t sample_bytes = (size_t)(MODE == MODE_CONVT ? p.Hout * p.Wout : p.Mh * p.Mw) * p.Cout * (RAW16 ? 2 : 4);
    const bool staged = FITS && stage != nullptr && sample_bytes < 0xfffffff0ull && (p.halo_tx != 0 || MODE == MODE_CONV);
    if constexpr (FITS) {
      if (staged) {
        if (has_cb) emit_whole_tile<BM, BN, MODE, RAW16, true, true, WR>(p, acc, tile_m, tile_n, cls, b, tid, cb_pre, use_pre, pivot, raw_mul, scl_s1, scl_s2, stage);
        else emit_whole_tile<BM, BN, MODE, RAW16, false, true, WR>(p, acc, tile_m, tile_n, cls, b, tid, cb_pre, use_pre, pivot, raw_mul, scl_s1, scl_s2, stage);
        return;
      }
    }
    if (has_cb) emit_whole_tile<BM, BN, MODE, RAW16, true, false, WR>(p, acc, tile_m, tile_n, cls, b, tid, cb_pre, use_pre, pivot, raw_mul, scl_s1, scl_s2, stage);
    else emit_whole_tile<BM, BN, MODE, RAW16, false, false, WR>(p, acc, tile_m, tile_n, cls, b, tid, cb_pre, use_pre, pivot, raw_mul, scl_s1, scl_s2, stage);
    return;
  }
#pragma unroll
  for (int i = 0; i < MT; ++i) {
    int m = tile_m * BM + wm * (MT * 32) + i * 32 + (lane & 31);
    if ((MODE == MODE_CONV || MODE == MODE_CONVT) && p.halo_tx) {
      const int local = wm * (MT * 32) + i * 32 + (lane & 31);
      const int tyi = (int)udiv_magic((unsigned)tile_m, (unsigned)p.halo_tx, p.mg_htx);
      m = halo_row(p, tyi, local >> 4, BM / 16) * p.Mw + (tile_m - tyi * p.halo_tx) * 16 + ((local & 15) ^ (((local >> 4) & 1) * p.halo_xor));
      if (!INTERIOR && (tile_m - tyi * p.halo_tx) * 16 + ((local & 15) ^ (((local >> 4) & 1) * p.halo_xor)) >= p.Mw) m = mtot;
    }
    const bool mok = INTERIOR || m < mtot;
    int mh = 0, mw = 0;
    if (MODE == MODE_CONVT || has_cb) {
      mh = (int)udiv_magic((unsigned)m, (unsigned)p.Mw, p.mg_mw);
      mw = m - mh * p.Mw;
    }
    size_t opix;
    bool sok = mok;
    if (MODE == MODE_CONVT) {
      int orow = 2 * mh + ph, ocol = 2 * mw + pw;
      if (wrapt) {
        orow -= 1; ocol -= 5;
        sok = mok && orow >= 0 && orow < p.Hout && ocol >= 0 && ocol < p.Wout;
      }
      opix = ((size_t)b * p.Hout + orow) * p.Wout + ocol;
    } else {
      opix = (size_t)b * mtot + m;
    }
    const float *cbrow = has_cb ? p.coord_bias + (size_t)(mh * COORD_CLASSES + coord_class(mw, p.Mw)) * p.cb_stride : nullptr;
    char *yrow = reinterpret_cast<char *>(p.y) + opix * p.Cout * YSZ;
#pragma unroll
    for (int j = 0; j < NT; ++j) {
      const int nb = tile_n * BN + wn * (NT * 32) + j * 32 + 4 * half;
#pragma unroll
      for (int g = 0; g < 4; ++g) {
        const int n = nb + 8 * g;
        const bool ok = mok && (INTERIOR || n < p.Cout);
        v4f v = {acc[i][j][4 * g], acc[i][j][4 * g + 1], acc[i][j][4 * g + 2], acc[i][j][4 * g + 3]};
        if (ok) {
          if (has_cb) {
            const v4f cb = (MT == 1 && NT == 1 && use_pre) ? cb_pre[g] : *reinterpret_cast<const v4f *>(cbrow + n);
            v.x += cb.x; v.y += cb.y; v.z += cb.z; v.w += cb.w;
          }
          if (MODE == MODE_HEAD) {
            const v4f bs = *reinterpret_cast<const v4f *>(p.bias + n);
            v.x = msi_tanh(v.x + bs.x); v.y = msi_tanh(v.y + bs.y); v.z = msi_tanh(v.z + bs.z); v.w = msi_tanh(v.w + bs.w);
          }
          if (sok && RAW16) {
            typedef _Float16 h2_t __attribute__((ext_vector_type(2)));
            typedef unsigned u2_t __attribute__((ext_vector_type(2)));
            const h2_t lo = {(_Float16)(v.x * raw_mul), (_Float16)(v.y * raw_mul)}, hi = {(_Float16)(v.z * raw_mul), (_Float16)(v.w * raw_mul)};
            *reinterpret_cast<u2_t *>(yrow + n * 2) = u2_t{__builtin_bit_cast(unsigned, lo), __builtin_bit_cast(unsigned, hi)};
          } else if (sok) {
            float *dst = reinterpret_cast<float *>(yrow) + n;
            if (vec_ok) {
              *reinterpret_cast<v4f *>(dst) = v;
            } else {
              dst[0] = v.x;
              if (n + 1 < p.Cout) dst[1] = v.y;
              if (n + 2 < p.Cout) dst[2] = v.z;
              if (n + 3 < p.Cout) dst[3] = v.w;
            }
          }
          if (want_stats) {
            const float dx = v.x - pivot, dy = v.y - pivot, dz = v.z - pivot, dw = v.w - pivot;
            if (INTERIOR || n + 3 < p.Cout) {
              s1 += (dx + dy) + (dz + dw);
              s2 += (dx * dx + dy * dy) + (dz * dz + dw * dw);
              cnt += 4.f;
            } else {
              s1 += dx; s2 += dx * dx; cnt += 1.f;
              if (n + 1 < p.Cout) { s1 += dy; s2 += dy * dy; cnt += 1.f; }
              if (n + 2 < p.Cout) { s1 += dz; s2 += dz * dz; cnt += 1.f; }
            }
          }
        }
      }
    }
  }
  if (want_stats) {
    s1 = wave_sum(s1);
    s2 = wave_sum(s2);
    const float wcnt = INTERIOR ? (float)(MT * NT * 16 * 64) : wave_sum(cnt);
    if (lane == 0 && wcnt > 0.f) {
      const double P = (double)pivot, n = (double)wcnt, a = (double)s1;
      long long *dst = p.sums + ((size_t)b * LN_SHARDS + ((blockIdx.x * 4 + wave) & (LN_SHARDS - 1))) * LN_WORDS;
      if (RAW16 && !(s2 * raw_mul * raw_mul <= 1.0727e9f)) __hip_atomic_fetch_or(p.status, STATUS_LN_OVERFLOW, __ATOMIC_RELAXED, __HIP_MEMORY_SCOPE_AGENT);
      ln_atomic_add(dst, (n * P + a) * scl_s1, p.status);
      ln_atomic_add(dst + 1, ((double)s2 + 2.0 * P * a + n * P * P) * scl_s2, p.status);
#if defined(MSI_DEBUG_STATS)
      if (p.dbg) {
        unsigned long long *o = p.dbg + 16384 * 24 + ((size_t)((blockIdx.x + gridDim.x * blockIdx.y) * 2 + (cls & 1)) * 4 + wave) * 4;
        o[0] = ((unsigned long long)__builtin_bit_cast(unsigned, s2) << 32) | __builtin_bit_cast(unsigned, s1);
        o[1] = ((unsigned long long)__builtin_bit_cast(unsigned, pivot) << 32) | __builtin_bit_cast(unsigned, wcnt);
        o[2] = __builtin_bit_cast(unsigned long long, (n * P + a) * scl_s1);
        o[3] = __builtin_bit_cast(unsigned long long, ((double)s2 + 2.0 * P * a + n * P * P) * scl_s2);
      }
#endif
    }
  }
}

template <int BM, int BN, int MODE, int RAW16 = 0, int WR = 2>
__device__ __forceinline__ void emit_tile(const ConvParams &p, f32x16 (&acc)[BM / (32 * WR)][BN / 64], int tile_m, int tile_n,
                                          int cls, int b, int tid, const v4f (&cb_pre)[4], bool use_pre, char *stage = nullptr,
                                          float raw_mul_pre = 0.f) {
  const bool interior = !(MODE == MODE_CONVT && p.wrap != 0) && (tile_m + 1) * BM <= p.Mh * p.Mw &&
                        (tile_n + 1) * BN <= p.Cout && (p.Cout & 3) == 0;
  if (interior) emit_tile_impl<BM, BN, MODE, true, RAW16, WR>(p, acc, tile_m, tile_n, cls, b, tid, cb_pre, use_pre, stage, raw_mul_pre);
  else emit_tile_impl<BM, BN, MODE, false, RAW16, WR>(p, acc, tile_m, tile_n, cls, b, tid, cb_pre, use_pre, nullptr, 0.f);
}
template <int BM, int BN, int MODE, int RAW16 = 0, int WR = 2>
__device__ __forceinline__ void emit_tile(const ConvParams &p, f32x16 (&acc)[BM / (32 * WR)][BN / 64], int tile_m, int tile_n,
                                          int cls, int b, int tid, char *stage = nullptr, float raw_mul_pre = 0.f) {
  const v4f none[4] = {};
  emit_tile<BM, BN, MODE, RAW16, WR>(p, acc, tile_m, tile_n, cls, b, tid, none, false, stage, raw_mul_pre);
}

__device__ __forceinline__ void load_coord_bias(const ConvParams &p, int tile_m, int tile_n, int tid, v4f (&cbv)[4]) {
#pragma unroll
  for (int g = 0; g < 4; ++g) cbv[g] = v4f{0.f, 0.f, 0.f, 0.f};
  if (p.coord_bias == nullptr) return;
  const int lane = tid & 63, wave = tid >> 6, wm = wave >> 1, wn = wave & 1, half = lane >> 5;
  int m = tile_m * 64 + wm * 32 + (lane & 31);
  if (p.halo_tx) {
    const int local = wm * 32 + (lane & 31);
    const int tyi = (int)udiv_magic((unsigned)tile_m, (unsigned)p.halo_tx, p.mg_htx);
    m = halo_row(p, tyi, local >> 4, 4) * p.Mw + (tile_m - tyi * p.halo_tx) * 16 + ((local & 15) ^ (((local >> 4) & 1) * p.halo_xor));
  }
  m = min(m, p.Mh * p.Mw - 1);
  const int mh = (int)udiv_magic((unsigned)m, (unsigned)p.Mw, p.mg_mw), mw = m - mh * p.Mw;
  const float *cbrow = p.coord_bias + (size_t)(mh * COORD_CLASSES + coord_class(mw, p.Mw)) * p.cb_stride;
#pragma unroll
  for (int g = 0; g < 4; ++g) {
    const int n = min(tile_n * 64 + wn * 32 + 4 * half + 8 * g, p.cb_stride - 4);
    cbv[g] = *reinterpret_cast<const v4f *>(cbrow + n);
  }
}

__device__ constexpr int s2_tap(int J) { return J == 0 ? 0 : J == 1 ? 2 : J == 2 ? 6 : J == 3 ? 8 : J == 4 ? 1 : J == 5 ? 7 : J == 6 ? 3 : J == 7 ? 5 : 4; }
__device__ constexpr int s2_unit(int J) { return J < 4 ? 0 : J < 6 ? 1 : J < 8 ? 2 : 3; }

}
```

### matryodshka_amd/csrc/cnn_plan.hip

```cpp
#include "cnn_plan.h"

namespace {

void plan_tiles(ConvParams &p, int BM, int BN, int batch, int num_cus, int tailsplit, int max_split, int *nblocks, int *nfix,
                int uniform_split = 0, int split_overhead = 0, bool split_any_tile = false) {
  const int mtot = p.Mh * p.Mw;
  p.tiles_m = (mtot + BM - 1) / BM;
  if (p.halo_tx) p.tiles_m = ((p.Mh + BM / 16 - 1) / (BM / 16)) * p.halo_tx;
  p.tiles_n = (p.Cout + BN - 1) / BN;
  p.ntiles = p.tiles_m * p.tiles_n * p.nclass * batch;
  p.n_main = p.ntiles;
  p.split0 = 1;
  p.split = 1;
  const int Q = CONV_SLOTS_PER_CU * num_cus;
  if (BM * BN == 64 * 64 && tailsplit == 2 && p.ntiles >= Q && p.ntiles % Q != 0 && p.ksteps >= 2 * MAX_SPLIT) {
    const int remq = p.ntiles % Q;
    int best = 1;
    double best_cost = 1.0;
    for (int sp = 2; sp <= max_split; ++sp) {
      if ((long)remq * sp > 2L * num_cus * MAX_SPLIT) break;
      const double cost = (double)((remq * sp + Q - 1) / Q) / sp;
      if (cost < best_cost - 1e-9) { best_cost = cost; best = sp; }
    }
    if (best > 1) { p.split = best; p.n_main = p.ntiles - remq; }
  }
  const bool uniform = uniform_split >= 2 && BM * BN == 64 * 64 && tailsplit && p.ntiles >= num_cus && p.ntiles < 2 * num_cus &&
                       uniform_split <= max_split && p.ksteps >= 2 * MAX_SPLIT;
  if (uniform) { p.n_main = 0; p.split0 = 1; p.split = uniform_split; }
  const int rem = p.ntiles % num_cus;
  if (!uniform && (BM * BN == 64 * 64 || split_any_tile) && p.split == 1 &&
      rem != 0 && p.ntiles > num_cus / 2 && p.ksteps >= 2 * MAX_SPLIT && tailsplit && !(tailsplit == 2 && p.ntiles >= Q)) {
    int best = 1;
    const double K = (double)p.ksteps, ovh = (double)split_overhead;
    double best_cost = K + ovh;
    for (int sp = 2; sp <= max_split; ++sp) {
      const double cost = (double)((rem * sp + num_cus - 1) / num_cus) * (K / sp + ovh);
      if (cost < best_cost - 1e-9) { best_cost = cost; best = sp; }
    }
    if (best > 1) { p.split = best; p.n_main = p.ntiles - rem; }
    if (p.n_main == num_cus && p.split > 1 && p.ksteps >= 4 * MAX_SPLIT && max_split >= 2) {
      p.split0 = 2;
      if (split_overhead == 0) p.split = p.split > 6 ? 6 : p.split;
    }
  }
  p.nb_main = p.n_main * p.split0;
  auto magic = [](int d) { return d == 1 ? 0xffffffffu : (unsigned)((1ull << 32) / (unsigned)d); };
  p.mg_mw = magic(p.Mw); p.mg_tm = magic(p.tiles_m); p.mg_tn = magic(p.tiles_n); p.mg_nc = magic(p.nclass);
  p.mg_sp0 = magic(p.split0);
  p.mg_sp = magic(p.split);
  *nblocks = p.nb_main + (p.ntiles - p.n_main) * p.split;
  *nfix = (p.split0 > 1 ? p.n_main : 0) + (p.split > 1 ? p.ntiles - p.n_main : 0);
}

enum { NO_CONVT_TILE8 = 1, NO_CONVT_HALO = 2 };

int choose_variant(const msi_net_plan *pl, int li, int exclude, ConvVariant &v, ConvParams &p) {
  const msi_net_desc *desc = &pl->desc;
  const Layer &L = pl->net.layers[li];
  const int bf16 = desc->dtype == MSI_DTYPE_BF16;
  int max_split = MAX_SPLIT;
  memset(&v, 0, sizeof(v));
  p.nclass = L.nclass;
  p.halo_tx = 0;
  const long tiles_big = (long)((L.mh * L.mw + 127) / 128) * ((L.cout + 127) / 128) * L.nclass * desc->batch;
  const int bigmode = pl->opt[MSI_NET_OPT_BIGTILE];
  v.family = CONV_IGEMM; v.bm = 64; v.bn = 64; v.mode = L.kind; v.bf16 = bf16;
  if (bf16 && L.cout % 128 == 0 && bigmode != 0 && (tiles_big >= 4L * pl->num_cus || bigmode == 2)) {
    v.bm = 128; v.bn = 128;
  } else if (bf16 && L.cout % 64 == 0 && bigmode != 0 && ((tiles_big >= 4L * pl->num_cus && L.cin <= 128) || bigmode == 2)) {
    v.bm = 128; v.bn = 64;
  }
  const bool tile64 = v.bm == 64 && v.bn == 64;
  const bool halo_ok = !((pl->opt[MSI_NET_OPT_HALO_SKIP] >> li) & 1);
  const bool x3_on = !bf16 && L.x3_off != 0 && ((pl->opt[MSI_NET_OPT_F32_SPLIT3] >> li) & 1);
  const int planes = ((pl->opt[MSI_NET_OPT_F32_SPLIT_F16] >> li) & 1) ? 2 : 3;
  const bool tile8_bit = (pl->opt[MSI_NET_OPT_X3_TILE8] >> li) & 1, tile8_force = (pl->opt[MSI_NET_OPT_X3_TILE8] >> 30) & 1;
  if (halo_ok && (pl->opt[MSI_NET_OPT_HALO] & 1) && !bf16 && tile64 &&
      L.kind == MODE_CONV && L.stride == 1 && L.src1 < 0 && L.in_h % 4 == 0 && L.in_w % 16 == 0 && L.c0 % 32 == 0 &&
      (L.rate == 1 || L.rate == 2)) {
    v.family = CONV_HALO; v.rate = L.rate;
    p.halo_tx = L.in_w / 16;
    if (x3_on) {
      v.family = CONV_HALO_X3; v.planes = planes;
      if (planes == 3 && L.rate == 1 && L.in_h % 8 == 0 && tile8_bit && ((long)(L.in_h / 8) * (L.in_w / 16) * ((L.cout + 63) / 64) * desc->batch >= 3L * pl->num_cus || tile8_force)) {
        v.family = CONV_HALO8_X3; v.bm = 128; v.rate = 0;
      }
      if (L.rate == 2 && L.in_h % 8 == 0 && ((pl->opt[MSI_NET_OPT_X3_ROWPAR] >> li) & 1)) v.rate = 3;
    }
  }
  if (halo_ok && (pl->opt[MSI_NET_OPT_HALO] & 4) && !bf16 && tile64 &&
      L.kind == MODE_CONV && L.stride == 2 && L.rate == 1 && L.src1 < 0 && L.in_h % 2 == 0 && L.in_w % 2 == 0 &&
      L.out_h % 4 == 0 && L.out_w % 16 == 0 && L.c0 % 32 == 0 && p.pad_t == p.pad_l && (p.pad_t == 0 || p.pad_t == 1) &&
      ((long)(L.out_h / 4) * (L.out_w / 16) * (L.cout / 64) * desc->batch >= 3L * pl->num_cus ||
       (L.x3_off != 0 && ((pl->opt[MSI_NET_OPT_F32_SPLIT3] >> li) & 1) && !(pl->opt[MSI_NET_OPT_HALO_SKIP] >> 20 & 1)))) {
    v.family = CONV_HALO_S2;
    p.halo_tx = L.out_w / 16;
    if (x3_on) {
      v.family = CONV_HALO_S2_X3; v.planes = planes;
      if (planes == 3 && L.out_h % 8 == 0 && tile8_bit && ((long)(L.out_h / 8) * (L.out_w / 16) * ((L.cout + 63) / 64) * desc->batch >= 3L * pl->num_cus || tile8_force)) {
        v.family = CONV_HALO8_S2_X3; v.bm = 128; v.planes = 0;
      }
    }
  }
  if (halo_ok && (pl->opt[MSI_NET_OPT_HALO] & 1) && bf16 && L.kind == MODE_CONV && L.stride == 1 && L.src1 < 0 && L.in_w % 16 == 0 &&
      L.c0 % 64 == 0 && bigmode != 0) {
    if (L.cout % 128 == 0 && L.in_h % 8 == 0 && (L.rate == 1 || L.rate == 2)) { v.family = CONV_HALO_BF16; v.bm = 128; v.bn = 128; v.rate = L.rate; v.waves = pl->opt[MSI_NET_OPT_BF16_WAVES] == 8 ? 8 : 4; }
    else if (L.cout == 64 && L.in_h % 16 == 0 && L.rate == 1) { v.family = CONV_HALO_BF16; v.bm = 256; v.bn = 64; v.rate = 1; v.waves = 4; }
    if (v.family == CONV_HALO_BF16) { p.halo_tx = L.in_w / 16; max_split = 1; }
  }
  if (halo_ok && (pl->opt[MSI_NET_OPT_HALO] & 4) && bf16 && L.kind == MODE_CONV && L.stride == 2 && L.rate == 1 &&
      L.src1 < 0 && L.in_h % 2 == 0 && L.in_w % 2 == 0 && L.out_h % 8 == 0 && L.out_w % 16 == 0 && L.c0 % 64 == 0 && L.cout % 128 == 0 &&
      p.pad_t == p.pad_l && (p.pad_t == 0 || p.pad_t == 1) && bigmode != 0) {
    v.family = CONV_HALO_BF16_S2; v.bm = 128; v.bn = 128; v.waves = 4; p.halo_tx = L.out_w / 16; max_split = 1;
  }
  if (!(exclude & NO_CONVT_HALO) &&
      halo_ok && ((pl->opt[MSI_NET_OPT_HALO] & 2) || (x3_on && pl->opt[MSI_NET_OPT_HALO] != 0)) && !bf16
      && tile64 && L.kind == MODE_CONVT && ((!L.wrapt && L.in_h % 4 == 0 && L.in_w % 16 == 0) || (L.wrapt && x3_on)) &&
      L.c0 % 32 == 0 && L.c1 % 32 == 0) {
    v.family = x3_on ? CONVT_HALO_X3 : CONVT_HALO; v.planes = x3_on ? planes : 0;
    p.nclass = 2;
    p.halo_tx = L.wrapt ? (L.mw + 15) / 16 : L.in_w / 16;
    if (L.cpt0 + L.cpt1 < max_split) max_split = L.cpt0 + L.cpt1;
    if (!(exclude & NO_CONVT_TILE8) && x3_on && planes == 3 && !L.wrapt && L.in_h % 8 == 0 && tile8_bit &&
        (2L * (L.in_h / 8) * (L.in_w / 16) * ((L.cout + 63) / 64) * desc->batch >= 3L * pl->num_cus || tile8_force)) {
      v.family = CONVT_HALO8_X3; v.bm = 128; v.planes = 0;
    }
  }
  if (halo_ok && (pl->opt[MSI_NET_OPT_HALO] & 1) && bf16 && L.kind == MODE_CONVT && !L.wrapt &&
      L.in_w % 16 == 0 && L.c0 % 64 == 0 && L.c1 % 64 == 0 && bigmode != 0) {
    if (L.cout % 128 == 0 && L.in_h % 8 == 0) { v.family = CONVT_HALO_BF16; v.bm = 128; v.bn = 128; }
    else if (L.cout == 64 && L.in_h % 8 == 0) { v.family = CONVT_HALO_BF16; v.bm = 128; v.bn = 64; }
    if (v.family == CONVT_HALO_BF16) { p.halo_tx = L.in_w / 16; p.nclass = 2; max_split = 1; }
  }
  if (v.is_halo()) {
    v.mode = 0; v.bf16 = 0;
    p.mg_htx = p.halo_tx == 1 ? 0xffffffffu : (unsigned)((1ull << 32) / (unsigned)p.halo_tx);
    if (!v.is_convt_f32() && L.cpt0 < max_split) max_split = L.cpt0;
  }
  p.halo_xor = (v.is_halo() && !bf16) ? 8 : 0;
  p.row_par = (v.family == CONV_HALO_X3 && v.rate == 3) ? 1 : 0;
  return max_split;
}

int plan_layers(msi_net_plan *pl) {
  const msi_net_desc *desc = &pl->desc;
  int rc = build_net(desc, pl->num_cus, pl->net);
  if (rc) return rc;
  const Net &net = pl->net;
  const int bf16 = desc->dtype == MSI_DTYPE_BF16;
  const int head_src = net.layers[MSI_NET_NUM_LAYERS - 1].src0;
  const bool fuse_head_ln = !bf16 && pl->opt[MSI_NET_OPT_HEAD_FUSE_LN] && net.layers[head_src].cout <= HEAD_MAX_C;
  for (int li = 0; li < MSI_NET_NUM_LAYERS; ++li) {
    const Layer &L = net.layers[li];
    LayerLaunch &Q = pl->launch[li];
    memset(&Q, 0, sizeof(Q));
    ConvParams &p = Q.p;
    ConvVariant &V = Q.variant;
    p.C0 = L.c0;
    p.C1 = L.src1 >= 0 ? L.c1 : 0;
    p.cb_stride = (int)round_up(L.cout, 4);
    p.Hin = L.in_h; p.Win = L.in_w; p.Hout = L.out_h; p.Wout = L.out_w;
    p.Cout = L.cout; p.npad = L.npad;
    p.ntaps = L.ntaps; p.cpt0 = L.cpt0; p.cpt1 = L.cpt1; p.ksteps = L.ksteps;
    p.mode = L.kind;
    p.wrap = desc->coord_net ? 0 : 1;
    p.rate = L.rate;
    p.Mh = L.mh; p.Mw = L.mw;
    p.stride = 1;
    if (L.kind == MODE_CONV) {
      p.stride = L.stride;
      if (desc->coord_net) {
        const int keff = 2 * L.rate + 1;
        const int th = (L.out_h - 1) * L.stride + keff - L.in_h, tw = (L.out_w - 1) * L.stride + keff - L.in_w;
        p.pad_t = (th > 0 ? th : 0) / 2;
        p.pad_l = (tw > 0 ? tw : 0) / 2;
      } else {
        p.pad_t = L.rate;
        p.pad_l = L.rate;
      }
    } else if (L.kind == MODE_CONVT && L.wrapt) {
      p.pad_t = 0;
      p.pad_l = 2;
    }
    if (L.kind == MODE_HEAD && fuse_head_ln) {
      Q.fuse_ln = 1;
      p.ln_inv_n = 1.0 / net.layers[L.src0].ln_count;
    }
    Q.skip_apply = fuse_head_ln && li == head_src;
    for (int exclude = 0;;) {
      const int max_split = choose_variant(pl, li, exclude, V, p);
      const bool tap_fallback = exclude & NO_CONVT_HALO;
      plan_tiles(p, V.bm, V.bn, desc->batch, pl->num_cus, pl->opt[MSI_NET_OPT_TAILSPLIT], max_split, &Q.nblocks, &Q.nfix,
                 tap_fallback ? 0 : pl->opt[MSI_NET_OPT_UNIFORM_SPLIT], tap_fallback ? 0 : pl->opt[MSI_NET_OPT_SPLIT_OVERHEAD], V.tile8());
      Q.inlaunch = !pl->opt[MSI_NET_OPT_FIXUP_KERNEL] && Q.nfix <= CONV_SLOTS_PER_CU * pl->num_cus;
      const size_t slab_bytes = (size_t)(Q.nblocks - (p.split0 == 1 ? p.nb_main : 0)) * (V.is_convt_f32() ? 2 : 1) * V.bm * V.bn * sizeof(float);
      if (slab_bytes <= net.partial_bytes) break;
      if (!V.is_convt_f32()) return msi::fail(MSI_E_WORKSPACE, "conv %s: %d partial accumulators exceed the workspace", L.name, Q.nblocks);
      exclude |= V.tile8() ? NO_CONVT_TILE8 : NO_CONVT_HALO;
    }
    if (L.kind != MODE_HEAD) {
      const size_t per_sample = (size_t)L.out_h * L.out_w * L.cout;
      size_t blocks = (per_sample / 4 + 255) / 256;
      if (blocks > 1024) blocks = 1024;
      Q.ln_blocks = (unsigned)blocks;
    }
  }
  for (int s = 0; s < MSI_NET_NUM_LAYERS - 1; ++s) {
    int consumers = 0, capable = 0;
    for (int li = s + 1; li < MSI_NET_NUM_LAYERS; ++li) {
      const Layer &L = net.layers[li];
      if (L.src0 == s || L.src1 == s) {
        ++consumers;
        const ConvVariant &C = pl->launch[li].variant;
        const int stage_raw = pl->opt[MSI_NET_OPT_BF16_STAGE_RAW];
        if (C.is_convt_f32() || (C.family == CONVT_HALO_BF16 && C.bn == 64 && (stage_raw & 2)) ||
            (C.is_halo() && !C.is_convt() && L.src0 == s && (!bf16 || (L.c0 <= 512 && (C.bm != 256 || (stage_raw & 1)))))) ++capable;
      }
    }
    if (consumers > 0 && consumers == capable) {
      pl->launch[s].skip_apply = 1;
      for (int li = s + 1; li < MSI_NET_NUM_LAYERS; ++li) {
        const Layer &L = net.layers[li];
        LayerLaunch &C = pl->launch[li];
        if (C.variant.is_convt()) {
          if (L.src0 == s) { C.p.halo_apply |= 1; C.p.ln_inv_n = 1.0 / net.layers[s].ln_count; }
          if (L.src1 == s) { C.p.halo_apply |= 2; C.p.ln_inv_n1 = 1.0 / net.layers[s].ln_count; }
          if ((L.src0 == s || L.src1 == s) && C.variant.family == CONVT_HALO_BF16) C.variant.apply = 1;
        } else if (L.src0 == s) {
          C.variant.apply = 1;
          C.p.ln_inv_n = 1.0 / net.layers[s].ln_count;
        }
      }
    }
  }
  return MSI_OK;
}

}

extern "C" {

int msi_net_plan_create(const msi_net_desc *desc, msi_net_plan **out) {
  MSI_REQUIRE(desc && out, "net_plan_create: null pointer");
  *out = nullptr;
  msi_net_plan *pl = new (std::nothrow) msi_net_plan();
  if (!pl) return msi::fail(MSI_E_WORKSPACE, "net_plan_create: out of host memory");
  pl->desc = *desc;
  pl->num_cus = device_cu_count();
  pl->opt[MSI_NET_OPT_FIXUP_KERNEL] = 0;
  pl->opt[MSI_NET_OPT_TAILSPLIT] = 1;
  pl->opt[MSI_NET_OPT_BIGTILE] = 1;
  pl->opt[MSI_NET_OPT_HEAD_FUSE_LN] = 1;
  pl->opt[MSI_NET_OPT_NUM_CUS] = pl->num_cus;
  pl->opt[MSI_NET_OPT_HALO] = 5;
  pl->opt[MSI_NET_OPT_UNIFORM_SPLIT] = 0;
  pl->opt[MSI_NET_OPT_SPLIT_OVERHEAD] = 0;
  pl->opt[MSI_NET_OPT_BF16_WAVES] = 8;
  pl->opt[MSI_NET_OPT_F32_SPLIT_F16] = 0;
  pl->opt[MSI_NET_OPT_X3_TILE8] = 0x3ffff;
  pl->opt[MSI_NET_OPT_X3_ROWPAR] = 0x3ffff;
  pl->opt[MSI_NET_OPT_F32_SPLIT3] = 0x3ffff;
  pl->opt[MSI_NET_OPT_BF16_STAGE_RAW] = 1;
  int rc = plan_layers(pl);
  if (rc) { delete pl; return rc; }
  *out = pl;
  return MSI_OK;
}

void msi_net_plan_destroy(msi_net_plan *plan) { delete plan; }

int msi_net_plan_set_option(msi_net_plan *plan, int32_t option, int32_t value) {
  MSI_REQUIRE(plan, "net_plan_set_option: null plan");
  MSI_REQUIRE(option >= 0 && option < MSI_NET_OPT_COUNT, "net_plan_set_option: unknown option %d", option);
  if (option == MSI_NET_OPT_F32_TILE || option == MSI_NET_OPT_F32_TILE_MASK || option == MSI_NET_OPT_APPLY_AHEAD) {
    if (option == MSI_NET_OPT_F32_TILE) MSI_REQUIRE(value >= 0 && value <= 2, "net_plan_set_option: f32 tile %d", value);
    if (value != 0) return msi::fail(MSI_E_UNSUPPORTED, "net_plan_set_option: option %d was an experiment (measured slower) whose code this library no longer has", option);
    return MSI_OK;
  }
  if (option == MSI_NET_OPT_NUM_CUS) {
    MSI_REQUIRE(value >= 8 && value <= 4096, "net_plan_set_option: num_cus %d out of range", value);
    plan->num_cus = value;
  }
  if (option == MSI_NET_OPT_BIGTILE) MSI_REQUIRE(value >= 0 && value <= 2, "net_plan_set_option: bigtile %d", value);
  if (option == MSI_NET_OPT_HALO) MSI_REQUIRE(value >= 0 && value <= 7, "net_plan_set_option: halo %d (bit 0 conv, bit 1 conv-transpose, bit 2 stride-2 conv)", value);
  if (option == MSI_NET_OPT_TAILSPLIT) MSI_REQUIRE(value >= 0 && value <= 2, "net_plan_set_option: tailsplit %d", value);
  if (option == MSI_NET_OPT_BF16_WAVES) MSI_REQUIRE(value == 4 || value == 8, "net_plan_set_option: bf16 waves %d (4 or 8)", value);
  const int old = plan->opt[option];
  plan->opt[option] = value;
  int rc = plan_layers(plan);
  if (rc) {
    plan->opt[option] = old;
    if (option == MSI_NET_OPT_NUM_CUS) plan->num_cus = old;
    plan_layers(plan);
  }
  return rc;
}

size_t msi_net_plan_workspace_bytes(const msi_net_plan *plan) { return plan ? plan->net.ws_bytes : 0; }

int32_t msi_net_plan_layer_is_normalized(const msi_net_plan *plan, int32_t layer) {
  if (!plan || layer < 0 || layer >= MSI_NET_NUM_LAYERS - 1) return -1;
  return plan->launch[layer].skip_apply ? 0 : 1;
}

int32_t msi_net_plan_layer_kernel(const msi_net_plan *plan, int32_t layer, char *name, size_t name_bytes, int32_t *nblocks,
                                  int32_t *nsplit_tiles) {
  MSI_REQUIRE(plan && name && name_bytes > 0, "net_plan_layer_kernel: null pointer");
  MSI_REQUIRE(layer >= 0 && layer < MSI_NET_NUM_LAYERS, "net_plan_layer_kernel: bad layer %d", layer);
  const LayerLaunch &Q = plan->launch[layer];
  const ConvVariant &V = Q.variant;
  switch (V.family) {
    case CONV_IGEMM: snprintf(name, name_bytes, "conv_igemm_kernel<%d, %d, %d, %d>", V.bm, V.bn, V.mode, V.bf16); break;
    case CONV_HALO: snprintf(name, name_bytes, "conv_halo_kernel<%d, %d>", V.rate, V.apply); break;
    case CONV_HALO_S2: snprintf(name, name_bytes, "conv_halo_s2_kernel<%d>", V.apply); break;
    case CONVT_HALO: snprintf(name, name_bytes, "convt_halo_kernel"); break;
    case CONV_HALO_X3: snprintf(name, name_bytes, "conv_halo_x3_kernel<%d, %d, %d>", V.rate, V.apply, V.planes); break;
    case CONV_HALO8_X3: snprintf(name, name_bytes, "conv_halo8_x3_kernel<%d, %d>", V.apply, V.planes); break;
    case CONV_HALO_S2_X3: snprintf(name, name_bytes, "conv_halo_s2_x3_kernel<%d, %d>", V.apply, V.planes); break;
    case CONV_HALO8_S2_X3: snprintf(name, name_bytes, "conv_halo8_s2_x3_kernel<%d>", V.apply); break;
    case CONVT_HALO_X3: snprintf(name, name_bytes, "convt_halo_x3_kernel<%d>", V.planes); break;
    case CONVT_HALO8_X3: snprintf(name, name_bytes, "convt_halo8_x3_kernel"); break;
    case CONV_HALO_BF16: snprintf(name, name_bytes, "conv_halo_bf16_kernel<%d, %d, %d, %d, %d>", V.bm, V.bn, V.rate, V.apply, V.waves); break;
    case CONV_HALO_BF16_S2: snprintf(name, name_bytes, "conv_halo_bf16_s2_kernel<%d, %d>", V.apply, V.waves); break;
    case CONVT_HALO_BF16: snprintf(name, name_bytes, "convt_halo_bf16_kernel<%d, %d, %d>", V.bm, V.bn, V.apply); break;
    default: return msi::fail(MSI_E_UNSUPPORTED, "net_plan_layer_kernel: unknown kernel family %d", V.family);
  }
  if (nblocks) *nblocks = Q.nblocks;
  if (nsplit_tiles) *nsplit_tiles = Q.nfix;
  return MSI_OK;
}

int32_t msi_net_plan_layer_params(const msi_net_plan *plan, int32_t layer, void *out, size_t bytes, size_t *needed) {
  MSI_REQUIRE(plan && (out || needed), "net_plan_layer_params: null pointer");
  MSI_REQUIRE(layer >= 0 && layer < MSI_NET_NUM_LAYERS, "net_plan_layer_params: bad layer %d", layer);
  const LayerLaunch &Q = plan->launch[layer];
  const int32_t tail[4] = {Q.inlaunch, Q.fuse_ln, Q.skip_apply, (int32_t)Q.ln_blocks};
  if (needed) *needed = sizeof(ConvParams) + sizeof(tail);
  if (!out) return MSI_OK;
  MSI_REQUIRE(bytes >= sizeof(ConvParams) + sizeof(tail), "net_plan_layer_params: %zu bytes, %zu needed", bytes, sizeof(ConvParams) + sizeof(tail));
  memcpy(out, &Q.p, sizeof(ConvParams));
  memcpy(static_cast<char *>(out) + sizeof(ConvParams), tail, sizeof(tail));
  return MSI_OK;
}

}
```

### matryodshka_amd/csrc/cnn_tail.hip

```cpp
#include "cnn_device.h"

namespace {


template <int BF16IN>
__global__ void __launch_bounds__(256) __attribute__((amdgpu_waves_per_eu(BF16IN ? 6 : 5)))
head_assemble_kernel(const HeadAsmParams p) {
  [[maybe_unused]] constexpr int FMT = MSI_LAYERS_F32;
#include "cnn_tail_head_assemble.inc"
}

template <int BF16IN, int FMT>
__global__ void __launch_bounds__(256) __attribute__((amdgpu_waves_per_eu(BF16IN ? 6 : 5)))
head_assemble_packed_kernel(const HeadAsmParams p) {
  static_assert(FMT == MSI_LAYERS_RGBA8 || FMT == MSI_LAYERS_RGBA16F, "a packed texel format");
#include "cnn_tail_head_assemble.inc"
}

__global__ void __launch_bounds__(256)
ln_finish_kernel(const long long *__restrict__ sums, double inv_n, const double *__restrict__ scl, int *status,
                 const float *__restrict__ gamma, const float *__restrict__ beta, int C, float *__restrict__ aff, int raw16) {
  __shared__ double s_stat[2];
  const int b = blockIdx.x, tid = threadIdx.x;
  ln_mean_inv(sums + (size_t)b * LN_SHARDS * LN_WORDS, inv_n, scl, status, s_stat, tid);
  const double mu = s_stat[0], inv = s_stat[1];
  const double up = raw16 ? scl[2] * 16777216.0 : 1.0;
  for (int c = tid; c < C; c += 256) {
    const double sc = inv * (double)gamma[c];
    aff[(size_t)b * 2 * C + c] = (float)(sc * up);
    aff[(size_t)b * 2 * C + C + c] = (float)((double)beta[c] - mu * sc);
  }
}

__global__ void __launch_bounds__(256) zero_kernel(float4 *__restrict__ p, size_t n16) {
  const size_t i = (size_t)blockIdx.x * 256 + threadIdx.x;
  if (i < n16) p[i] = float4{0.f, 0.f, 0.f, 0.f};
}

template <int BF16OUT>
__global__ void __launch_bounds__(256)
ln_apply_kernel(float *__restrict__ x, const long long *__restrict__ sums, double inv_n, const double *__restrict__ scl,
                int *status, const float *__restrict__ gamma, const float *__restrict__ beta, size_t per_sample, int C,
                float *__restrict__ aff, unsigned short *__restrict__ yb) {
  extern __shared__ __attribute__((aligned(16))) float s_aff[];
  __shared__ double s_stat[2];
  const int b = blockIdx.y, tid = threadIdx.x;
  ln_mean_inv(sums + (size_t)b * LN_SHARDS * LN_WORDS, inv_n, scl, (blockIdx.x == 0 ? status : nullptr), s_stat, tid);
  const double mu = s_stat[0], inv = s_stat[1];
  const double up = BF16OUT ? scl[2] * 16777216.0 : 1.0;
  for (int c = tid; c < C; c += 256) {
    const double sc = inv * (double)gamma[c];
    const float fs = (float)sc, ft = (float)((double)beta[c] - mu * sc);
    s_aff[c] = BF16OUT ? (float)(sc * up) : fs;
    s_aff[C + c] = ft;
    if (blockIdx.x == 0) {
      aff[(size_t)b * 2 * C + c] = fs;
      aff[(size_t)b * 2 * C + C + c] = ft;
    }
  }
  __syncthreads();

  typedef _Float16 h4_t __attribute__((ext_vector_type(4)));
  const h4_t *xh = reinterpret_cast<const h4_t *>(reinterpret_cast<const _Float16 *>(x) + (size_t)b * per_sample);
  v4f *xv = reinterpret_cast<v4f *>(x + (size_t)b * per_sample);
  auto get = [&](size_t i) __attribute__((always_inline)) -> v4f {
    if (BF16OUT == 1) { const h4_t h = xh[i]; return v4f{(float)h.x, (float)h.y, (float)h.z, (float)h.w}; }
    return xv[i];
  };
  const size_t nvec = per_sample / 4;
  const size_t stride = (size_t)gridDim.x * blockDim.x;
  auto apply = [](v4f v, const v4f s4, const v4f t4) __attribute__((always_inline)) -> v4f {
    v.x = fmaxf(v.x * s4.x + t4.x, 0.f);
    v.y = fmaxf(v.y * s4.y + t4.y, 0.f);
    v.z = fmaxf(v.z * s4.z + t4.z, 0.f);
    v.w = fmaxf(v.w * s4.w + t4.w, 0.f);
    return v;
  };
  auto bf16_bits = [](float f) __attribute__((always_inline)) -> unsigned {
    const unsigned u = __builtin_bit_cast(unsigned, f);
    return (u + 0x7fffu + ((u >> 16) & 1u)) >> 16;
  };
  typedef unsigned v2u __attribute__((ext_vector_type(2)));
  v2u *yv = reinterpret_cast<v2u *>(yb + (size_t)b * per_sample);
  auto put = [&](size_t i, const v4f v) __attribute__((always_inline)) {
    if (BF16OUT == 1) yv[i] = v2u{bf16_bits(v.x) | (bf16_bits(v.y) << 16), bf16_bits(v.z) | (bf16_bits(v.w) << 16)};
    else xv[i] = v;
  };
  if ((256 * 4) % C == 0) {
    const int c = (tid * 4) % C;
    const v4f s4 = *reinterpret_cast<const v4f *>(s_aff + c);
    const v4f t4 = *reinterpret_cast<const v4f *>(s_aff + C + c);
    for (size_t i = (size_t)blockIdx.x * blockDim.x + tid; i < nvec; i += stride) put(i, apply(get(i), s4, t4));
  } else {
    for (size_t i = (size_t)blockIdx.x * blockDim.x + tid; i < nvec; i += stride) {
      const int c = (int)((i * 4) % C);
      put(i, apply(get(i), *reinterpret_cast<const v4f *>(s_aff + c), *reinterpret_cast<const v4f *>(s_aff + C + c)));
    }
  }
}

}

namespace msi_cnn {
int launch_zero(void *ptr, size_t n16, hipStream_t stream) {
  hipLaunchKernelGGL(zero_kernel, dim3((unsigned)((n16 + 255) / 256)), dim3(256), 0, stream, reinterpret_cast<float4 *>(ptr), n16);
  return msi::check_launch("zero");
}
int launch_ln_finish(int batch, hipStream_t stream, const long long *sums, double inv_n, const double *scl, int *status, const float *gamma, const float *beta, int C,
                     float *aff, int raw16) {
  hipLaunchKernelGGL(ln_finish_kernel, dim3(batch), dim3(256), 0, stream, sums, inv_n, scl, status, gamma, beta, C, aff, raw16);
  return msi::check_launch("ln_finish");
}
int launch_ln_apply(int bf16out, unsigned blocks, int batch, size_t lds, hipStream_t stream, float *x, const long long *sums, double inv_n, const double *scl, int *status,
                    const float *gamma, const float *beta, size_t per_sample, int C, float *aff, unsigned short *yb) {
  const dim3 grid(blocks, batch);
  if (bf16out) hipLaunchKernelGGL(ln_apply_kernel<1>, grid, dim3(256), lds, stream, x, sums, inv_n, scl, status, gamma, beta, per_sample, C, aff, yb);
  else hipLaunchKernelGGL(ln_apply_kernel<0>, grid, dim3(256), lds, stream, x, sums, inv_n, scl, status, gamma, beta, per_sample, C, aff, yb);
  return msi::check_launch("ln_apply");
}
int launch_head_assemble(int bf16in, int format, unsigned grid_x, size_t lds, hipStream_t stream, const HeadAsmParams &q) {
#define MSI_LAUNCH_HA(K) hipLaunchKernelGGL(K, dim3(grid_x), dim3(256), lds, stream, q)
  switch (format) {
    case MSI_LAYERS_F32:
      if (bf16in) MSI_LAUNCH_HA(head_assemble_kernel<1>); else MSI_LAUNCH_HA(head_assemble_kernel<0>);
      break;
    case MSI_LAYERS_RGBA8:
      if (bf16in) MSI_LAUNCH_HA((head_assemble_packed_kernel<1, MSI_LAYERS_RGBA8>)); else MSI_LAUNCH_HA((head_assemble_packed_kernel<0, MSI_LAYERS_RGBA8>));
      break;
    case MSI_LAYERS_RGBA16F:
      if (bf16in) MSI_LAUNCH_HA((head_assemble_packed_kernel<1, MSI_LAYERS_RGBA16F>)); else MSI_LAUNCH_HA((head_assemble_packed_kernel<0, MSI_LAYERS_RGBA16F>));
      break;
    default:
      return msi::fail(MSI_E_BADARG, "head_assemble: unknown format %d", format);
  }
#undef MSI_LAUNCH_HA
  return msi::check_launch("head_assemble");
}
}
```

### matryodshka_amd/csrc/cnn_tail_head_assemble.inc

```
#if defined(__HIP_DEVICE_COMPILE__)
  extern __shared__ __attribute__((aligned(16))) char smem[];
  constexpr int BN = 64;
  const int tid = threadIdx.x, lane = tid & 63, wave = tid >> 6;
  const int nd = p.nd, lg = p.lg, ng = p.ng;
  const unsigned slot = blockIdx.x >> 3;
  const unsigned tsl = ng == 1 ? slot : (ng == 2 ? slot >> 1 : slot / (unsigned)ng);
  const int g = (int)(slot - tsl * (unsigned)ng);
  const long tile = (long)tsl * 8 + (blockIdx.x & 7u);
  if (tile * HA_TP >= p.npix_total) return;
  const int c_psv = 6 * nd, c_pred = 2 * nd;
  const int l_cpsv = 6 * lg, l_cpred = 2 * lg;
  const int s_psv = l_cpsv + 1, s_pred = l_cpred + 1;
  const int s_psv16 = 3 * lg + 1;
  float *s_aff = reinterpret_cast<float *>(smem);
  char *sR = smem + 2 * 64 * 4 + 64;
  char *sA = sR;
  char *sB = sA + p.ksteps * HA_TP * ROW_BYTES;
  const size_t r_bytes = BF16IN ? max((size_t)p.ksteps * HA_TP * ROW_BYTES, (size_t)HA_TP * s_psv16 * sizeof(unsigned))
                                : max((size_t)p.ksteps * (HA_TP + BN) * ROW_BYTES, (size_t)HA_TP * s_psv * sizeof(float));
  float *l_psv = reinterpret_cast<float *>(sR);
  float *l_pred = reinterpret_cast<float *>(sR + ((r_bytes + 15) & ~(size_t)15));
  auto gcol = [&](int n) __attribute__((always_inline)) -> int { return n < lg ? g * lg + n : nd + g * lg + (n - lg); };

  const long p0 = tile * HA_TP;
  const int b = (int)udiv_magic((unsigned)p0, (unsigned)p.hw, p.mg_hw);
  constexpr int PSV_PER_THREAD = BF16IN ? 3 : 6;
  constexpr int B_PER_THREAD = 4;
  constexpr int PSV_VEC = BF16IN ? 8 : 4;
  constexpr int ESZ = BF16IN ? 2 : 4;
  const int nrun = ng == 1 ? 1 : 2;
  const int run_len = ng == 1 ? c_psv : 3 * lg;
  const int vpr = run_len / PSV_VEC, vpp = nrun * vpr;
  const int nv_psv = HA_TP * vpp;
  float4 q[PSV_PER_THREAD];
  {
    const char *gp = static_cast<const char *>(p.psv) + (size_t)p0 * c_psv * ESZ;
#pragma unroll
    for (int k = 0; k < PSV_PER_THREAD; ++k) {
      const int v = tid + 256 * k;
      if (v < nv_psv) {
        if (ng == 1) {
          q[k] = reinterpret_cast<const float4 *>(gp)[v];
        } else {
          const int px = (int)udiv_magic((unsigned)v, (unsigned)vpp, p.mg_vpp), w = v - px * vpp;
          const int r = w >= vpr ? 1 : 0, idx = w - r * vpr;
          const int start = r == 0 ? 3 * g * lg : 3 * (nd + g * lg);
          q[k] = *reinterpret_cast<const float4 *>(gp + ((size_t)px * c_psv + start + idx * PSV_VEC) * ESZ);
        }
      }
    }
  }
  const int nchunk = p.ksteps * 8;
  v4f araw[2];
  if (BF16IN) {
    typedef _Float16 h8_t __attribute__((ext_vector_type(8)));
    const int r = tid >> 3, c = (tid & 7) * 8;
    araw[0] = araw[1] = v4f{0.f, 0.f, 0.f, 0.f};
    if (c < p.C0) {
      const h8_t h = *reinterpret_cast<const h8_t *>(reinterpret_cast<const _Float16 *>(p.x) + (size_t)(p0 + r) * p.C0 + c);
      araw[0] = v4f{(float)h[0], (float)h[1], (float)h[2], (float)h[3]};
      araw[1] = v4f{(float)h[4], (float)h[5], (float)h[6], (float)h[7]};
    }
  } else {
#pragma unroll
    for (int k = 0; k < 2; ++k) {
      const int e = tid + 256 * k;
      const int r = (int)udiv_magic((unsigned)e, (unsigned)nchunk, p.mg_nchunk), c = (e - r * nchunk) * 4;
      araw[k] = v4f{0.f, 0.f, 0.f, 0.f};
      if (e < HA_TP * nchunk && c < p.C0) araw[k] = *reinterpret_cast<const v4f *>(p.x + (size_t)(p0 + r) * p.C0 + c);
    }
  }
  const int nb = p.ksteps * BN * 8;
  v4f braw[B_PER_THREAD];
  v4f wfrag[4];
  if (BF16IN) {
    if (wave < 2) {
      const int frow = lane & 31, fh = lane >> 5;
      const int nloc = wave * 32 + frow;
      const int gn = gcol(nloc < l_cpred ? nloc : 0);
      const int fswz = (gn >> 1) & 7;
#pragma unroll
      for (int qq = 0; qq < 4; ++qq) {
        wfrag[qq] = v4f{0.f, 0.f, 0.f, 0.f};
        if (nloc < l_cpred)
          wfrag[qq] = *reinterpret_cast<const v4f *>(p.wpk + (size_t)gn * (ROW_BYTES / 4) + (((2 * qq + fh) ^ fswz) << 2));
      }
    }
  } else {
#pragma unroll
    for (int k = 0; k < B_PER_THREAD; ++k) {
      const int e = tid + 256 * k;
      const int row = e >> 3, j = e & 7;
      const int ks = row / BN, n = row - ks * BN;
      braw[k] = v4f{0.f, 0.f, 0.f, 0.f};
      if (e < nb && n < l_cpred)
        braw[k] = *reinterpret_cast<const v4f *>(p.wpk + ((size_t)ks * p.npad + gcol(n)) * (ROW_BYTES / 4) + j * 4);
    }
  }
  if (tid < 2 * p.C0) s_aff[tid] = p.aff[(size_t)b * 2 * p.C0 + tid];
  __syncthreads();
  if (BF16IN) {
    const int r = tid >> 3, ch = tid & 7, c = ch * 8;
    unsigned pk[4] = {0u, 0u, 0u, 0u};
    if (c < p.C0) {
      float y[8];
#pragma unroll
      for (int k = 0; k < 2; ++k) {
        const v4f s4 = *reinterpret_cast<const v4f *>(s_aff + c + 4 * k), t4 = *reinterpret_cast<const v4f *>(s_aff + p.C0 + c + 4 * k);
        y[4 * k] = fmaxf(araw[k].x * s4.x + t4.x, 0.f); y[4 * k + 1] = fmaxf(araw[k].y * s4.y + t4.y, 0.f);
        y[4 * k + 2] = fmaxf(araw[k].z * s4.z + t4.z, 0.f); y[4 * k + 3] = fmaxf(araw[k].w * s4.w + t4.w, 0.f);
      }
#pragma unroll
      for (int k = 0; k < 4; ++k) asm("v_cvt_pk_bf16_f32 %0, %1, %2" : "=v"(pk[k]) : "v"(y[2 * k]), "v"(y[2 * k + 1]));
    }
    typedef unsigned v4u_t __attribute__((ext_vector_type(4)));
    *reinterpret_cast<v4u_t *>(sA + r * ROW_BYTES + ((ch ^ ((r >> 1) & 7)) << 4)) = v4u_t{pk[0], pk[1], pk[2], pk[3]};
  } else
#pragma unroll
  for (int k = 0; k < 2; ++k) {
    const int e = tid + 256 * k;
    if (e < HA_TP * nchunk) {
      const int r = (int)udiv_magic((unsigned)e, (unsigned)nchunk, p.mg_nchunk), ch = e - r * nchunk;
      const int c = ch * 4;
      v4f y = {0.f, 0.f, 0.f, 0.f};
      if (c < p.C0) {
        const v4f s4 = *reinterpret_cast<const v4f *>(s_aff + c), t4 = *reinterpret_cast<const v4f *>(s_aff + p.C0 + c);
        y.x = fmaxf(araw[k].x * s4.x + t4.x, 0.f); y.y = fmaxf(araw[k].y * s4.y + t4.y, 0.f);
        y.z = fmaxf(araw[k].z * s4.z + t4.z, 0.f); y.w = fmaxf(araw[k].w * s4.w + t4.w, 0.f);
      }
      const int ks = ch >> 3, chunk = ch & 7;
      *reinterpret_cast<v4f *>(sA + (ks * HA_TP + r) * ROW_BYTES + ((chunk ^ ((r >> 1) & 7)) << 4)) = y;
    }
  }
  if (!BF16IN) {
#pragma unroll
    for (int k = 0; k < B_PER_THREAD; ++k) {
      const int e = tid + 256 * k;
      if (e < nb) *reinterpret_cast<v4f *>(sB + (e >> 3) * ROW_BYTES + ((e & 7) << 4)) = braw[k];
    }
  }
  __syncthreads();
  if (wave < 2) {
    f32x16 acc;
#pragma unroll
    for (int r = 0; r < 16; ++r) acc[r] = 0.f;
    const int frow = lane & 31, fh = lane >> 5;
    const int fswz_a = (frow >> 1) & 7;
    const int fswz_b = (gcol(wave * 32 + frow < l_cpred ? wave * 32 + frow : 0) >> 1) & 7;
    if (BF16IN) {
      typedef __bf16 bf16x8 __attribute__((ext_vector_type(8)));
#pragma unroll
      for (int qq = 0; qq < 4; ++qq) {
        const v4f a = *reinterpret_cast<const v4f *>(sA + frow * ROW_BYTES + (((2 * qq + fh) ^ fswz_a) << 4));
        acc = __builtin_amdgcn_mfma_f32_32x32x16_bf16(__builtin_bit_cast(bf16x8, wfrag[qq]), __builtin_bit_cast(bf16x8, a), acc, 0, 0, 0);
      }
    } else
    for (int ks = 0; ks < p.ksteps; ++ks) {
#pragma unroll
      for (int qq = 0; qq < 4; ++qq) {
        const v4f a = *reinterpret_cast<const v4f *>(sA + (ks * HA_TP + frow) * ROW_BYTES + (((fh * 4 + qq) ^ fswz_a) << 4));
        const v4f w = *reinterpret_cast<const v4f *>(sB + (ks * BN + wave * 32 + frow) * ROW_BYTES + (((fh * 4 + qq) ^ fswz_b) << 4));
        acc = __builtin_amdgcn_mfma_f32_32x32x2f32(w.x, a.x, acc, 0, 0, 0);
        acc = __builtin_amdgcn_mfma_f32_32x32x2f32(w.y, a.y, acc, 0, 0, 0);
        acc = __builtin_amdgcn_mfma_f32_32x32x2f32(w.z, a.z, acc, 0, 0, 0);
        acc = __builtin_amdgcn_mfma_f32_32x32x2f32(w.w, a.w, acc, 0, 0, 0);
      }
    }
    const int px = lane & 31, half = lane >> 5;
#pragma unroll
    for (int gg = 0; gg < 4; ++gg) {
      const int n = wave * 32 + 8 * gg + 4 * half;
      if (n < l_cpred) {
        const int gn = gcol(n);
        const v4f bs = *reinterpret_cast<const v4f *>(p.bias + gn);
        v4f t = {msi_tanh(acc[4 * gg] + bs.x), msi_tanh(acc[4 * gg + 1] + bs.y), msi_tanh(acc[4 * gg + 2] + bs.z), msi_tanh(acc[4 * gg + 3] + bs.w)};
        if (p.pred_out) *reinterpret_cast<v4f *>(p.pred_out + (p0 + px) * c_pred + gn) = t;
        t.x = (t.x + 1.0f) / 2.0f; t.y = (t.y + 1.0f) / 2.0f; t.z = (t.z + 1.0f) / 2.0f; t.w = (t.w + 1.0f) / 2.0f;
        float *dst = l_pred + px * s_pred + n;
        dst[0] = t.x; dst[1] = t.y; dst[2] = t.z; dst[3] = t.w;
        if (n < lg) {
          if (p.bw_out) *reinterpret_cast<v4f *>(p.bw_out + (p0 + px) * nd + gn) = t;
        } else {
          if (p.al_out) *reinterpret_cast<v4f *>(p.al_out + (p0 + px) * nd + (gn - nd)) = t;
        }
      }
    }
  }
  __syncthreads();
#pragma unroll
  for (int k = 0; k < PSV_PER_THREAD; ++k) {
    const int v = tid + 256 * k;
    if (v < nv_psv) {
      const int px = (int)udiv_magic((unsigned)v, (unsigned)vpp, p.mg_vpp), w = v - px * vpp;
      if (BF16IN) {
        unsigned *dst = reinterpret_cast<unsigned *>(l_psv) + px * s_psv16 + w * 4;
        dst[0] = __builtin_bit_cast(unsigned, q[k].x); dst[1] = __builtin_bit_cast(unsigned, q[k].y);
        dst[2] = __builtin_bit_cast(unsigned, q[k].z); dst[3] = __builtin_bit_cast(unsigned, q[k].w);
      } else {
        float *dst = l_psv + px * s_psv + w * PSV_VEC;
        dst[0] = q[k].x; dst[1] = q[k].y; dst[2] = q[k].z; dst[3] = q[k].w;
      }
    }
  }
  __syncthreads();
  {
#pragma clang fp contract(off)
    const int px = tid & (HA_TP - 1);
    const long pp = p0 + px;
    const long off = pp - (long)b * p.hw;
    const float *rp = l_psv + px * s_psv;
    const float *rq = l_pred + px * s_pred;
    float4 *dst = p.rgba + ((long)b * nd + g * lg + tid / HA_TP) * p.hw + off;
    const long dstep = (long)(256 / HA_TP) * p.hw;
    constexpr int TEXEL_BYTES = FMT == MSI_LAYERS_RGBA8 ? 4 : 8;
    char *dstp = FMT != MSI_LAYERS_F32 ? static_cast<char *>(p.layers) + (((long)b * nd + g * lg + tid / HA_TP) * p.hw + off) * TEXEL_BYTES : nullptr;
    const bool want_f32 = FMT == MSI_LAYERS_F32 || p.rgba != nullptr;
    const unsigned *rp16 = reinterpret_cast<const unsigned *>(l_psv) + px * s_psv16;
    for (int d = tid / HA_TP; d < lg; d += 256 / HA_TP, dst += dstep, dstp += dstep * TEXEL_BYTES) {
      float fgv[3], bgv[3];
      if (BF16IN) {
        const int ef = 3 * d, eb = 3 * (lg + d);
        const unsigned f0 = rp16[ef >> 1], f1 = rp16[(ef >> 1) + 1], b0 = rp16[eb >> 1], b1 = rp16[(eb >> 1) + 1];
        const unsigned long long fw = ((unsigned long long)f1 << 32 | f0) >> ((ef & 1) * 16), bw = ((unsigned long long)b1 << 32 | b0) >> ((eb & 1) * 16);
#pragma unroll
        for (int c = 0; c < 3; ++c) {
          fgv[c] = __builtin_bit_cast(float, (unsigned)(fw >> (16 * c)) << 16);
          bgv[c] = __builtin_bit_cast(float, (unsigned)(bw >> (16 * c)) << 16);
        }
      } else {
#pragma unroll
        for (int c = 0; c < 3; ++c) { fgv[c] = rp[d * 3 + c]; bgv[c] = rp[(lg + d) * 3 + c]; }
      }
      const float *fg = fgv;
      const float *bg = bgv;
      const float w = rq[d];
      const float omw = 1.0f - w;
      float4 o;
      o.x = w * fg[0] + omw * bg[0];
      o.y = w * fg[1] + omw * bg[1];
      o.z = w * fg[2] + omw * bg[2];
      o.w = rq[lg + d];
      if constexpr (FMT == MSI_LAYERS_RGBA8) *reinterpret_cast<unsigned *>(dstp) = rgba8_encode(o);
      else if constexpr (FMT == MSI_LAYERS_RGBA16F) *reinterpret_cast<u32x2_g *>(dstp) = rgba16f_encode(o);
      if (want_f32) {
#if defined(MSI_HA_NT) && MSI_HA_NT
        __builtin_nontemporal_store(o.x, &dst->x); __builtin_nontemporal_store(o.y, &dst->y); __builtin_nontemporal_store(o.z, &dst->z); __builtin_nontemporal_store(o.w, &dst->w);
#else
        *dst = o;
#endif
      }
    }
  }
#endif
```

Before: 547.0.

## Add 64-pixel fp32 fused head-assemble tail with 512-thread workgroups

Templates the fused head/assemble tail kernel on pixels per workgroup and adds a 64-pixel, 512-thread variant for fp32 plans. It is the default when H*W divides by 64. Four GEMM waves now split the tile by pixel block and column block, and bias loads are hoisted ahead of the barrier. Weight loads become branch-free with zero-fill applied at the LDS store. The larger tile spreads the weight staging over more pixels and halves the workgroup count, at the cost of more LDS per workgroup, a lower waves-per-EU target, and possibly an opt-in for more than 64 KiB of LDS.

```diff
diff --git a/include/msi_hip.h b/include/msi_hip.h
--- a/include/msi_hip.h
+++ b/include/msi_hip.h
@@ -238,7 +238,8 @@
 #define MSI_NET_OPT_F32_SPLIT_F16 15
 #define MSI_NET_OPT_X3_TILE8 16
 #define MSI_NET_OPT_X3_ROWPAR 17
-#define MSI_NET_OPT_COUNT 18
+#define MSI_NET_OPT_TAIL_TP 18
+#define MSI_NET_OPT_COUNT 19
 int msi_net_plan_create(const msi_net_desc *desc, msi_net_plan **out_plan);
 void msi_net_plan_destroy(msi_net_plan *plan);
 int msi_net_plan_set_option(msi_net_plan *plan, int32_t option, int32_t value);
diff --git a/matryodshka_amd/_native.py b/matryodshka_amd/_native.py
--- a/matryodshka_amd/_native.py
+++ b/matryodshka_amd/_native.py
@@ -33,6 +33,7 @@
 NET_OPT_F32_SPLIT_F16 = 15
 NET_OPT_X3_TILE8 = 16
 NET_OPT_X3_ROWPAR = 17
+NET_OPT_TAIL_TP = 18
 NET_STATUS_F16_SPLIT_RANGE = 8
 
 
diff --git a/matryodshka_amd/csrc/cnn.hip b/matryodshka_amd/csrc/cnn.hip
--- a/matryodshka_amd/csrc/cnn.hip
+++ b/matryodshka_amd/csrc/cnn.hip
@@ -38,6 +38,15 @@
 extern "C" void msi_debug_conv_timing(void *device_buffer, int layer) {
   g_timing_buf = static_cast<unsigned long long *>(device_buffer);
   g_timing_layer = layer;
+}
+#endif
+
+#ifdef MSI_HA_STAMP
+static unsigned long long *g_ha_stamp_buf = nullptr;
+static int g_ha_stamp_blocks = 0;
+extern "C" void msi_debug_ha_stamps(void *device_buffer, int blocks) {
+  g_ha_stamp_buf = static_cast<unsigned long long *>(device_buffer);
+  g_ha_stamp_blocks = blocks;
 }
 #endif
 
@@ -238,11 +247,16 @@
   const int bf16 = desc->dtype == MSI_DTYPE_BF16;
   if ((!bf16 && !plan->launch[MSI_NET_NUM_LAYERS - 1].fuse_ln) || (bf16 && !plan->opt[MSI_NET_OPT_HEAD_FUSE_LN]) ||
       H.c0 > 64 || H.c0 % 4 != 0 || desc->num_outputs != 2 * nd || nd % 4 != 0 || nd > 64 || desc->in_channels != 6 * nd ||
-      ((long)desc->height * desc->width) % HA_TP != 0)
+      ((long)desc->height * desc->width) % HA_TP_MIN != 0)
     return msi::fail(MSI_E_UNSUPPORTED, "%s: fused tail needs a blend_psv network (in = 6 D, out = 2 D, "
                      "D %% 4 == 0, D <= 64, ngf <= 64, HEAD_FUSE_LN on)", who);
   MSI_REQUIRE(rgba_native || layers_out, "%s: null pointer", who);
   MSI_REQUIRE(!layers_out || (reinterpret_cast<uintptr_t>(layers_out) & 15) == 0, "%s: layers_out is not 16-byte aligned", who);
+  const long hw_px = (long)desc->height * desc->width;
+  const int tp_opt = plan->opt[MSI_NET_OPT_TAIL_TP];
+  if (tp_opt == HA_TP_MAX && (bf16 || hw_px % HA_TP_MAX != 0))
+    return msi::fail(MSI_E_UNSUPPORTED, "%s: the 64-pixel fused tail needs an fp32 plan and H * W %% 64 == 0", who);
+  const int tp = tp_opt ? tp_opt : (!bf16 && hw_px % HA_TP_MAX == 0 ? HA_TP_MAX : HA_TP_MIN);
   const int ng = (nd + HA_LG - 1) / HA_LG;
   if (nd % ng != 0 || (nd / ng) % 4 != 0 || (ng > 1 && bf16 && (nd / ng) % 8 != 0))
     return msi::fail(MSI_E_UNSUPPORTED, "%s: D = %d does not split into layer groups of a multiple of %d", who, nd, bf16 ? 8 : 4);
@@ -286,16 +300,19 @@
     if (q.npix_total >= (1L << 32)) return msi::fail(MSI_E_UNSUPPORTED, "%s: more than 2^32 pixels per batch", who);
   }
   constexpr int BN = 64;
-  size_t r_bytes = (size_t)q.ksteps * (HA_TP + BN) * ROW_BYTES;
-  if (r_bytes < (size_t)HA_TP * (6 * q.lg + 1) * sizeof(float)) r_bytes = (size_t)HA_TP * (6 * q.lg + 1) * sizeof(float);
+  size_t r_bytes = (size_t)q.ksteps * (tp + BN) * ROW_BYTES;
+  if (r_bytes < (size_t)tp * (6 * q.lg + 1) * sizeof(float)) r_bytes = (size_t)tp * (6 * q.lg + 1) * sizeof(float);
   if (bf16) {
-    r_bytes = (size_t)q.ksteps * HA_TP * ROW_BYTES;
-    if (r_bytes < (size_t)HA_TP * (3 * q.lg + 1) * sizeof(unsigned)) r_bytes = (size_t)HA_TP * (3 * q.lg + 1) * sizeof(unsigned);
-  }
-  const size_t lds = 2 * 64 * 4 + 64 + ((r_bytes + 15) & ~(size_t)15) + (size_t)HA_TP * (2 * q.lg + 1) * sizeof(float);
-  const long ntile = q.npix_total / HA_TP;
+    r_bytes = (size_t)q.ksteps * tp * ROW_BYTES;
+    if (r_bytes < (size_t)tp * (3 * q.lg + 1) * sizeof(unsigned)) r_bytes = (size_t)tp * (3 * q.lg + 1) * sizeof(unsigned);
+  }
+  const size_t lds = 2 * 64 * 4 + 64 + ((r_bytes + 15) & ~(size_t)15) + (size_t)tp * (2 * q.lg + 1) * sizeof(float);
+  const long ntile = q.npix_total / tp;
   if (((ntile + 7) / 8) * 8 * ng >= (1L << 31)) return msi::fail(MSI_E_UNSUPPORTED, "%s: too many pixel tiles for one launch", who);
-  return launch_head_assemble(bf16, layers_out ? format : MSI_LAYERS_F32, (unsigned)(((ntile + 7) / 8) * 8 * ng), lds, stream, q);
+#ifdef MSI_HA_STAMP
+  q.dbg = g_ha_stamp_buf; q.dbg_blocks = g_ha_stamp_blocks;
+#endif
+  return launch_head_assemble(bf16, layers_out ? format : MSI_LAYERS_F32, tp, (unsigned)(((ntile + 7) / 8) * 8 * ng), lds, stream, q);
 }
 
 int msi_net_plan_forward_rgba(const msi_net_plan *plan, const float *packed, const void *net_input, float *rgba_native,
diff --git a/matryodshka_amd/csrc/cnn_device.h b/matryodshka_amd/csrc/cnn_device.h
--- a/matryodshka_amd/csrc/cnn_device.h
+++ b/matryodshka_amd/csrc/cnn_device.h
@@ -110,11 +110,12 @@
   unsigned ln_blocks;
 };
 
-constexpr int HA_TP = 32;
+constexpr int HA_TP_MIN = 32, HA_TP_MAX = 64;
 #ifndef MSI_HA_LG
 #define MSI_HA_LG 32
 #endif
 constexpr int HA_LG = MSI_HA_LG;
+constexpr int HA_MAX_LDS = 2 * 64 * 4 + 64 + ((HA_TP_MAX * (6 * HA_LG + 1) * 4 + 15) & ~15) + HA_TP_MAX * (2 * HA_LG + 1) * 4;
 
 struct HeadAsmParams {
   const float *x;
@@ -130,6 +131,10 @@
   unsigned mg_vpp, mg_nchunk, mg_hw;
   long npix_total;
   void *layers;
+#ifdef MSI_HA_STAMP
+  unsigned long long *dbg;
+  int dbg_blocks;
+#endif
 };
 
 int launch_conv(const LayerLaunch &Q, const ConvParams &p, hipStream_t stream);
@@ -143,7 +148,7 @@
                      float *aff, int raw16);
 int launch_ln_apply(int bf16out, unsigned blocks, int batch, size_t lds, hipStream_t stream, float *x, const long long *sums, double inv_n, const double *scl, int *status,
                     const float *gamma, const float *beta, size_t per_sample, int C, float *aff, unsigned short *yb);
-int launch_head_assemble(int bf16in, int format, unsigned grid_x, size_t lds, hipStream_t stream, const HeadAsmParams &q);
+int launch_head_assemble(int bf16in, int format, int tp, unsigned grid_x, size_t lds, hipStream_t stream, const HeadAsmParams &q);
 int debug_conv_occupancy(int lds_bytes);
 
 constexpr int vkey(int family, int a = 0, int b = 0, int c = 0, int d = 0, int e = 0) { return ((((family * 16 + a) * 16 + b) * 16 + c) * 16 + d) * 16 + e; }
diff --git a/matryodshka_amd/csrc/cnn_plan.hip b/matryodshka_amd/csrc/cnn_plan.hip
--- a/matryodshka_amd/csrc/cnn_plan.hip
+++ b/matryodshka_amd/csrc/cnn_plan.hip
@@ -256,6 +256,7 @@
   pl->opt[MSI_NET_OPT_UNIFORM_SPLIT] = 0;
   pl->opt[MSI_NET_OPT_SPLIT_OVERHEAD] = 0;
   pl->opt[MSI_NET_OPT_BF16_WAVES] = 8;
+  pl->opt[MSI_NET_OPT_TAIL_TP] = 0;
   pl->opt[MSI_NET_OPT_F32_SPLIT_F16] = 0;
   pl->opt[MSI_NET_OPT_X3_TILE8] = 0x3ffff;
   pl->opt[MSI_NET_OPT_X3_ROWPAR] = 0x3ffff;
@@ -285,6 +286,11 @@
   if (option == MSI_NET_OPT_HALO) MSI_REQUIRE(value >= 0 && value <= 7, "net_plan_set_option: halo %d (bit 0 conv, bit 1 conv-transpose, bit 2 stride-2 conv)", value);
   if (option == MSI_NET_OPT_TAILSPLIT) MSI_REQUIRE(value >= 0 && value <= 2, "net_plan_set_option: tailsplit %d", value);
   if (option == MSI_NET_OPT_BF16_WAVES) MSI_REQUIRE(value == 4 || value == 8, "net_plan_set_option: bf16 waves %d (4 or 8)", value);
+  if (option == MSI_NET_OPT_TAIL_TP) {
+    MSI_REQUIRE(value == 0 || value == 32 || value == 64, "net_plan_set_option: tail tp %d (0, 32 or 64 pixels per workgroup)", value);
+    if (value == 64 && plan->desc.dtype == MSI_DTYPE_BF16)
+      return msi::fail(MSI_E_UNSUPPORTED, "net_plan_set_option: the fused tail of a bf16 plan has no 64-pixel form");
+  }
   const int old = plan->opt[option];
   plan->opt[option] = value;
   int rc = plan_layers(plan);
diff --git a/matryodshka_amd/csrc/cnn_tail.hip b/matryodshka_amd/csrc/cnn_tail.hip
--- a/matryodshka_amd/csrc/cnn_tail.hip
+++ b/matryodshka_amd/csrc/cnn_tail.hip
@@ -3,15 +3,15 @@
 namespace {
 
 
-template <int BF16IN>
-__global__ void __launch_bounds__(256) __attribute__((amdgpu_waves_per_eu(BF16IN ? 6 : 5)))
+template <int BF16IN, int TP>
+__global__ void __launch_bounds__(8 * TP) __attribute__((amdgpu_waves_per_eu(BF16IN ? 6 : 4)))
 head_assemble_kernel(const HeadAsmParams p) {
   [[maybe_unused]] constexpr int FMT = MSI_LAYERS_F32;
 #include "cnn_tail_head_assemble.inc"
 }
 
-template <int BF16IN, int FMT>
-__global__ void __launch_bounds__(256) __attribute__((amdgpu_waves_per_eu(BF16IN ? 6 : 5)))
+template <int BF16IN, int FMT, int TP>
+__global__ void __launch_bounds__(8 * TP) __attribute__((amdgpu_waves_per_eu(BF16IN ? 6 : 4)))
 head_assemble_packed_kernel(const HeadAsmParams p) {
   static_assert(FMT == MSI_LAYERS_RGBA8 || FMT == MSI_LAYERS_RGBA16F, "a packed texel format");
 #include "cnn_tail_head_assemble.inc"
@@ -118,22 +118,34 @@
   else hipLaunchKernelGGL(ln_apply_kernel<0>, grid, dim3(256), lds, stream, x, sums, inv_n, scl, status, gamma, beta, per_sample, C, aff, yb);
   return msi::check_launch("ln_apply");
 }
-int launch_head_assemble(int bf16in, int format, unsigned grid_x, size_t lds, hipStream_t stream, const HeadAsmParams &q) {
-#define MSI_LAUNCH_HA(K) hipLaunchKernelGGL(K, dim3(grid_x), dim3(256), lds, stream, q)
+template <auto KERNEL, int TP>
+static int launch_ha(unsigned grid_x, size_t lds, hipStream_t stream, const HeadAsmParams &q) {
+  if (lds > 65536) {
+    static thread_local unsigned long long done = 0;
+    int rc0 = set_max_lds(reinterpret_cast<const void *>(KERNEL), HA_MAX_LDS, done, "head_assemble");
+    if (rc0) return rc0;
+  }
+  hipLaunchKernelGGL(KERNEL, dim3(grid_x), dim3(8 * TP), lds, stream, q);
+  return msi::check_launch("head_assemble");
+}
+
+int launch_head_assemble(int bf16in, int format, int tp, unsigned grid_x, size_t lds, hipStream_t stream, const HeadAsmParams &q) {
+  if ((tp != 32 && tp != 64) || (bf16in && tp != 32) || lds > (size_t)HA_MAX_LDS)
+    return msi::fail(MSI_E_UNSUPPORTED, "head_assemble: no kernel for %d pixels per workgroup (%s, format %d, %zu bytes of LDS)", tp, bf16in ? "bf16" : "fp32", format, lds);
   switch (format) {
     case MSI_LAYERS_F32:
-      if (bf16in) MSI_LAUNCH_HA(head_assemble_kernel<1>); else MSI_LAUNCH_HA(head_assemble_kernel<0>);
-      break;
+      if (bf16in) return launch_ha<head_assemble_kernel<1, 32>, 32>(grid_x, lds, stream, q);
+      return tp == 64 ? launch_ha<head_assemble_kernel<0, 64>, 64>(grid_x, lds, stream, q) : launch_ha<head_assemble_kernel<0, 32>, 32>(grid_x, lds, stream, q);
     case MSI_LAYERS_RGBA8:
-      if (bf16in) MSI_LAUNCH_HA((head_assemble_packed_kernel<1, MSI_LAYERS_RGBA8>)); else MSI_LAUNCH_HA((head_assemble_packed_kernel<0, MSI_LAYERS_RGBA8>));
-      break;
+      if (bf16in) return launch_ha<head_assemble_packed_kernel<1, MSI_LAYERS_RGBA8, 32>, 32>(grid_x, lds, stream, q);
+      return tp == 64 ? launch_ha<head_assemble_packed_kernel<0, MSI_LAYERS_RGBA8, 64>, 64>(grid_x, lds, stream, q)
+                      : launch_ha<head_assemble_packed_kernel<0, MSI_LAYERS_RGBA8, 32>, 32>(grid_x, lds, stream, q);
     case MSI_LAYERS_RGBA16F:
-      if (bf16in) MSI_LAUNCH_HA((head_assemble_packed_kernel<1, MSI_LAYERS_RGBA16F>)); else MSI_LAUNCH_HA((head_assemble_packed_kernel<0, MSI_LAYERS_RGBA16F>));
-      break;
+      if (bf16in) return launch_ha<head_assemble_packed_kernel<1, MSI_LAYERS_RGBA16F, 32>, 32>(grid_x, lds, stream, q);
+      return tp == 64 ? launch_ha<head_assemble_packed_kernel<0, MSI_LAYERS_RGBA16F, 64>, 64>(grid_x, lds, stream, q)
+                      : launch_ha<head_assemble_packed_kernel<0, MSI_LAYERS_RGBA16F, 32>, 32>(grid_x, lds, stream, q);
     default:
       return msi::fail(MSI_E_BADARG, "head_assemble: unknown format %d", format);
   }
-#undef MSI_LAUNCH_HA
-  return msi::check_launch("head_assemble");
 }
 }
diff --git a/matryodshka_amd/csrc/cnn_tail_head_assemble.inc b/matryodshka_amd/csrc/cnn_tail_head_assemble.inc
--- a/matryodshka_amd/csrc/cnn_tail_head_assemble.inc
+++ b/matryodshka_amd/csrc/cnn_tail_head_assemble.inc
@@ -1,13 +1,20 @@
 #if defined(__HIP_DEVICE_COMPILE__)
   extern __shared__ __attribute__((aligned(16))) char smem[];
   constexpr int BN = 64;
+  constexpr int NT = 8 * TP;
+  static_assert(TP == 32 || (TP == 64 && !BF16IN), "32 pixels, or 64 on the fp32 head");
   const int tid = threadIdx.x, lane = tid & 63, wave = tid >> 6;
+#ifdef MSI_HA_STAMP
+  const unsigned long long ha_t0 = __builtin_amdgcn_s_memtime();
+#endif
+  const bool gemm_wave = wave < TP / 16;
+  const int pb = TP == 32 ? 0 : wave >> 1, cb = TP == 32 ? wave : wave & 1;
   const int nd = p.nd, lg = p.lg, ng = p.ng;
   const unsigned slot = blockIdx.x >> 3;
   const unsigned tsl = ng == 1 ? slot : (ng == 2 ? slot >> 1 : slot / (unsigned)ng);
   const int g = (int)(slot - tsl * (unsigned)ng);
   const long tile = (long)tsl * 8 + (blockIdx.x & 7u);
-  if (tile * HA_TP >= p.npix_total) return;
+  if (tile * TP >= p.npix_total) return;
   const int c_psv = 6 * nd, c_pred = 2 * nd;
   const int l_cpsv = 6 * lg, l_cpred = 2 * lg;
   const int s_psv = l_cpsv + 1, s_pred = l_cpred + 1;
@@ -15,29 +22,29 @@
   float *s_aff = reinterpret_cast<float *>(smem);
   char *sR = smem + 2 * 64 * 4 + 64;
   char *sA = sR;
-  char *sB = sA + p.ksteps * HA_TP * ROW_BYTES;
-  const size_t r_bytes = BF16IN ? max((size_t)p.ksteps * HA_TP * ROW_BYTES, (size_t)HA_TP * s_psv16 * sizeof(unsigned))
-                                : max((size_t)p.ksteps * (HA_TP + BN) * ROW_BYTES, (size_t)HA_TP * s_psv * sizeof(float));
+  char *sB = sA + p.ksteps * TP * ROW_BYTES;
+  const size_t r_bytes = BF16IN ? max((size_t)p.ksteps * TP * ROW_BYTES, (size_t)TP * s_psv16 * sizeof(unsigned))
+                                : max((size_t)p.ksteps * (TP + BN) * ROW_BYTES, (size_t)TP * s_psv * sizeof(float));
   float *l_psv = reinterpret_cast<float *>(sR);
   float *l_pred = reinterpret_cast<float *>(sR + ((r_bytes + 15) & ~(size_t)15));
   auto gcol = [&](int n) __attribute__((always_inline)) -> int { return n < lg ? g * lg + n : nd + g * lg + (n - lg); };
 
-  const long p0 = tile * HA_TP;
+  const long p0 = tile * TP;
   const int b = (int)udiv_magic((unsigned)p0, (unsigned)p.hw, p.mg_hw);
   constexpr int PSV_PER_THREAD = BF16IN ? 3 : 6;
-  constexpr int B_PER_THREAD = 4;
+  constexpr int B_PER_THREAD = 1024 / NT;
   constexpr int PSV_VEC = BF16IN ? 8 : 4;
   constexpr int ESZ = BF16IN ? 2 : 4;
   const int nrun = ng == 1 ? 1 : 2;
   const int run_len = ng == 1 ? c_psv : 3 * lg;
   const int vpr = run_len / PSV_VEC, vpp = nrun * vpr;
-  const int nv_psv = HA_TP * vpp;
+  const int nv_psv = TP * vpp;
   float4 q[PSV_PER_THREAD];
   {
     const char *gp = static_cast<const char *>(p.psv) + (size_t)p0 * c_psv * ESZ;
 #pragma unroll
     for (int k = 0; k < PSV_PER_THREAD; ++k) {
-      const int v = tid + 256 * k;
+      const int v = tid + NT * k;
       if (v < nv_psv) {
         if (ng == 1) {
           q[k] = reinterpret_cast<const float4 *>(gp)[v];
@@ -64,19 +71,19 @@
   } else {
 #pragma unroll
     for (int k = 0; k < 2; ++k) {
-      const int e = tid + 256 * k;
+      const int e = tid + NT * k;
       const int r = (int)udiv_magic((unsigned)e, (unsigned)nchunk, p.mg_nchunk), c = (e - r * nchunk) * 4;
       araw[k] = v4f{0.f, 0.f, 0.f, 0.f};
-      if (e < HA_TP * nchunk && c < p.C0) araw[k] = *reinterpret_cast<const v4f *>(p.x + (size_t)(p0 + r) * p.C0 + c);
+      if (e < TP * nchunk && c < p.C0) araw[k] = *reinterpret_cast<const v4f *>(p.x + (size_t)(p0 + r) * p.C0 + c);
     }
   }
   const int nb = p.ksteps * BN * 8;
   v4f braw[B_PER_THREAD];
   v4f wfrag[4];
   if (BF16IN) {
-    if (wave < 2) {
+    if (gemm_wave) {
       const int frow = lane & 31, fh = lane >> 5;
-      const int nloc = wave * 32 + frow;
+      const int nloc = cb * 32 + frow;
       const int gn = gcol(nloc < l_cpred ? nloc : 0);
       const int fswz = (gn >> 1) & 7;
 #pragma unroll
@@ -89,12 +96,20 @@
   } else {
 #pragma unroll
     for (int k = 0; k < B_PER_THREAD; ++k) {
-      const int e = tid + 256 * k;
+      const int e = tid + NT * k;
       const int row = e >> 3, j = e & 7;
       const int ks = row / BN, n = row - ks * BN;
-      braw[k] = v4f{0.f, 0.f, 0.f, 0.f};
-      if (e < nb && n < l_cpred)
-        braw[k] = *reinterpret_cast<const v4f *>(p.wpk + ((size_t)ks * p.npad + gcol(n)) * (ROW_BYTES / 4) + j * 4);
+      const bool ok = e < nb && n < l_cpred;
+      braw[k] = *reinterpret_cast<const v4f *>(p.wpk + ((size_t)(ok ? ks : 0) * p.npad + gcol(ok ? n : 0)) * (ROW_BYTES / 4) + j * 4);
+    }
+  }
+  v4f bsv[4];
+  if (!BF16IN && gemm_wave) {
+#pragma unroll
+    for (int gg = 0; gg < 4; ++gg) {
+      const int n = cb * 32 + 8 * gg + 4 * (lane >> 5);
+      bsv[gg] = v4f{0.f, 0.f, 0.f, 0.f};
+      if (n < l_cpred) bsv[gg] = *reinterpret_cast<const v4f *>(p.bias + gcol(n));
     }
   }
   if (tid < 2 * p.C0) s_aff[tid] = p.aff[(size_t)b * 2 * p.C0 + tid];
@@ -118,8 +133,8 @@
   } else
 #pragma unroll
   for (int k = 0; k < 2; ++k) {
-    const int e = tid + 256 * k;
-    if (e < HA_TP * nchunk) {
+    const int e = tid + NT * k;
+    if (e < TP * nchunk) {
       const int r = (int)udiv_magic((unsigned)e, (unsigned)nchunk, p.mg_nchunk), ch = e - r * nchunk;
       const int c = ch * 4;
       v4f y = {0.f, 0.f, 0.f, 0.f};
@@ -129,24 +144,27 @@
         y.z = fmaxf(araw[k].z * s4.z + t4.z, 0.f); y.w = fmaxf(araw[k].w * s4.w + t4.w, 0.f);
       }
       const int ks = ch >> 3, chunk = ch & 7;
-      *reinterpret_cast<v4f *>(sA + (ks * HA_TP + r) * ROW_BYTES + ((chunk ^ ((r >> 1) & 7)) << 4)) = y;
+      *reinterpret_cast<v4f *>(sA + (ks * TP + r) * ROW_BYTES + ((chunk ^ ((r >> 1) & 7)) << 4)) = y;
     }
   }
   if (!BF16IN) {
 #pragma unroll
     for (int k = 0; k < B_PER_THREAD; ++k) {
-      const int e = tid + 256 * k;
-      if (e < nb) *reinterpret_cast<v4f *>(sB + (e >> 3) * ROW_BYTES + ((e & 7) << 4)) = braw[k];
-    }
-  }
-  __syncthreads();
-  if (wave < 2) {
+      const int e = tid + NT * k;
+      if (e < nb) *reinterpret_cast<v4f *>(sB + (e >> 3) * ROW_BYTES + ((e & 7) << 4)) = ((e >> 3) % BN) >= l_cpred ? v4f{0.f, 0.f, 0.f, 0.f} : braw[k];
+    }
+  }
+  __syncthreads();
+#ifdef MSI_HA_STAMP
+  const unsigned long long ha_t1 = __builtin_amdgcn_s_memtime();
+#endif
+  if (gemm_wave) {
     f32x16 acc;
 #pragma unroll
     for (int r = 0; r < 16; ++r) acc[r] = 0.f;
     const int frow = lane & 31, fh = lane >> 5;
     const int fswz_a = (frow >> 1) & 7;
-    const int fswz_b = (gcol(wave * 32 + frow < l_cpred ? wave * 32 + frow : 0) >> 1) & 7;
+    const int fswz_b = (gcol(cb * 32 + frow < l_cpred ? cb * 32 + frow : 0) >> 1) & 7;
     if (BF16IN) {
       typedef __bf16 bf16x8 __attribute__((ext_vector_type(8)));
 #pragma unroll
@@ -158,21 +176,21 @@
     for (int ks = 0; ks < p.ksteps; ++ks) {
 #pragma unroll
       for (int qq = 0; qq < 4; ++qq) {
-        const v4f a = *reinterpret_cast<const v4f *>(sA + (ks * HA_TP + frow) * ROW_BYTES + (((fh * 4 + qq) ^ fswz_a) << 4));
-        const v4f w = *reinterpret_cast<const v4f *>(sB + (ks * BN + wave * 32 + frow) * ROW_BYTES + (((fh * 4 + qq) ^ fswz_b) << 4));
+        const v4f a = *reinterpret_cast<const v4f *>(sA + (ks * TP + pb * 32 + frow) * ROW_BYTES + (((fh * 4 + qq) ^ fswz_a) << 4));
+        const v4f w = *reinterpret_cast<const v4f *>(sB + (ks * BN + cb * 32 + frow) * ROW_BYTES + (((fh * 4 + qq) ^ fswz_b) << 4));
         acc = __builtin_amdgcn_mfma_f32_32x32x2f32(w.x, a.x, acc, 0, 0, 0);
         acc = __builtin_amdgcn_mfma_f32_32x32x2f32(w.y, a.y, acc, 0, 0, 0);
         acc = __builtin_amdgcn_mfma_f32_32x32x2f32(w.z, a.z, acc, 0, 0, 0);
         acc = __builtin_amdgcn_mfma_f32_32x32x2f32(w.w, a.w, acc, 0, 0, 0);
       }
     }
-    const int px = lane & 31, half = lane >> 5;
+    const int px = pb * 32 + (lane & 31), half = lane >> 5;
 #pragma unroll
     for (int gg = 0; gg < 4; ++gg) {
-      const int n = wave * 32 + 8 * gg + 4 * half;
+      const int n = cb * 32 + 8 * gg + 4 * half;
       if (n < l_cpred) {
         const int gn = gcol(n);
-        const v4f bs = *reinterpret_cast<const v4f *>(p.bias + gn);
+        const v4f bs = BF16IN ? *reinterpret_cast<const v4f *>(p.bias + gn) : bsv[gg];
         v4f t = {msi_tanh(acc[4 * gg] + bs.x), msi_tanh(acc[4 * gg + 1] + bs.y), msi_tanh(acc[4 * gg + 2] + bs.z), msi_tanh(acc[4 * gg + 3] + bs.w)};
         if (p.pred_out) *reinterpret_cast<v4f *>(p.pred_out + (p0 + px) * c_pred + gn) = t;
         t.x = (t.x + 1.0f) / 2.0f; t.y = (t.y + 1.0f) / 2.0f; t.z = (t.z + 1.0f) / 2.0f; t.w = (t.w + 1.0f) / 2.0f;
@@ -186,10 +204,17 @@
       }
     }
   }
+#ifdef MSI_HA_STAMP
+  if (p.dbg && lane == 0 && (int)blockIdx.x < p.dbg_blocks) {
+    unsigned long long *o = p.dbg + ((size_t)blockIdx.x * 8 + wave) * 4;
+    o[0] = (unsigned long long)__builtin_amdgcn_s_getreg(4 | (31 << 11)) | (unsigned long long)(__builtin_amdgcn_s_getreg(20 | (31 << 11)) & 0xf) << 32 | (gemm_wave ? 1ull << 40 : 0ull);
+    o[1] = ha_t0; o[2] = ha_t1; o[3] = __builtin_amdgcn_s_memtime();
+  }
+#endif
   __syncthreads();
 #pragma unroll
   for (int k = 0; k < PSV_PER_THREAD; ++k) {
-    const int v = tid + 256 * k;
+    const int v = tid + NT * k;
     if (v < nv_psv) {
       const int px = (int)udiv_magic((unsigned)v, (unsigned)vpp, p.mg_vpp), w = v - px * vpp;
       if (BF16IN) {
@@ -205,18 +230,18 @@
   __syncthreads();
   {
 #pragma clang fp contract(off)
-    const int px = tid & (HA_TP - 1);
+    const int px = tid & (TP - 1);
     const long pp = p0 + px;
     const long off = pp - (long)b * p.hw;
     const float *rp = l_psv + px * s_psv;
     const float *rq = l_pred + px * s_pred;
-    float4 *dst = p.rgba + ((long)b * nd + g * lg + tid / HA_TP) * p.hw + off;
-    const long dstep = (long)(256 / HA_TP) * p.hw;
+    float4 *dst = p.rgba + ((long)b * nd + g * lg + tid / TP) * p.hw + off;
+    const long dstep = (long)(NT / TP) * p.hw;
     constexpr int TEXEL_BYTES = FMT == MSI_LAYERS_RGBA8 ? 4 : 8;
-    char *dstp = FMT != MSI_LAYERS_F32 ? static_cast<char *>(p.layers) + (((long)b * nd + g * lg + tid / HA_TP) * p.hw + off) * TEXEL_BYTES : nullptr;
+    char *dstp = FMT != MSI_LAYERS_F32 ? static_cast<char *>(p.layers) + (((long)b * nd + g * lg + tid / TP) * p.hw + off) * TEXEL_BYTES : nullptr;
     const bool want_f32 = FMT == MSI_LAYERS_F32 || p.rgba != nullptr;
     const unsigned *rp16 = reinterpret_cast<const unsigned *>(l_psv) + px * s_psv16;
-    for (int d = tid / HA_TP; d < lg; d += 256 / HA_TP, dst += dstep, dstp += dstep * TEXEL_BYTES) {
+    for (int d = tid / TP; d < lg; d += NT / TP, dst += dstep, dstp += dstep * TEXEL_BYTES) {
       float fgv[3], bgv[3];
       if (BF16IN) {
         const int ef = 3 * d, eb = 3 * (lg + d);
```

New measurement: 550.3 (median of 6 runs). No clear change (+0.6%).
